# pytorch/torchsnapshot

Measured on AMD Instinct MI355X. Metric: checkpoint_save_GBps, higher is better.
Workload: dtype bf16; 1 GPU; model=llama-3-8b, model_bytes=16060522496, parallelism=fsdp1, storage=/tmp/tsamd_bench

## Files before the change

### torchsnapshot_amd/batcher.py

```python

from __future__ import annotations

import asyncio
from collections import defaultdict
from typing import Dict, List, Optional, Sequence

import torch

from . import knobs
from .io_types import (
    BufferConsumer,
    BufferStager,
    BufferType,
    ReadReq,
    StageContext,
    WriteReq,
)
from .io_preparers.tensor import TensorBufferStager
from .ops.staging import ALIGN, build_pack_items, get_pinned_pool, get_staging_engine
from .serialization import SERIALIZER_BUFFER


def _is_batchable(req: WriteReq) -> bool:
    stager = req.stager
    return (
        req.tensor_entry is not None
        and isinstance(stager, TensorBufferStager)
        and stager.serializer == SERIALIZER_BUFFER
        and not stager.tensor.is_quantized
        and stager.get_staging_cost_bytes() < knobs.get_slab_size_threshold_bytes()
    )


def batch_write_requests(
    write_reqs: List[WriteReq], rank: int = 0
) -> List[WriteReq]:
    if knobs.is_batching_disabled():
        return write_reqs
    out: List[WriteReq] = []
    groups: Dict[str, List[WriteReq]] = defaultdict(list)
    for req in write_reqs:
        if _is_batchable(req):
            groups[str(req.stager.tensor.device)].append(req)
        else:
            out.append(req)

    slab_limit = knobs.get_slab_size_threshold_bytes()
    seq = 0
    for device_str, members in groups.items():
        if len(members) == 1:
            out.extend(members)
            continue
        cur: List[WriteReq] = []
        cur_bytes = 0
        for req in members:
            nbytes = req.stager.stored_nbytes()
            aligned = (nbytes + ALIGN - 1) // ALIGN * ALIGN
            if cur and cur_bytes + aligned > slab_limit:
                out.append(_make_slab(device_str, cur, rank, seq))
                seq += 1
                cur, cur_bytes = [], 0
            cur.append(req)
            cur_bytes += aligned
        if len(cur) == 1:
            out.append(cur[0])
        elif cur:
            out.append(_make_slab(device_str, cur, rank, seq))
            seq += 1
    return out


def _make_slab(
    device_str: str, members: List[WriteReq], rank: int, seq: int
) -> WriteReq:
    slab_path = f"batched/{rank}-{seq}"
    tensors = [m.stager.tensor.detach() for m in members]
    out_dtypes = [m.stager.save_dtype for m in members]
    _, offsets, total = build_pack_items(tensors, out_dtypes)
    for m, off in zip(members, offsets):
        entry = m.tensor_entry
        nbytes = m.stager.stored_nbytes()
        entry.location = slab_path
        entry.byte_range = [off, off + nbytes]
    is_async = any(m.stager.is_async_snapshot for m in members)
    stager = BatchedBufferStager(
        tensors=tensors,
        total_bytes=total,
        is_async_snapshot=is_async,
        out_dtypes=out_dtypes,
    )
    return WriteReq(path=slab_path, stager=stager)


class BatchedBufferStager(BufferStager):
    def __init__(
        self,
        tensors: Sequence[torch.Tensor],
        total_bytes: int,
        is_async_snapshot: bool,
        out_dtypes: Optional[Sequence[Optional[torch.dtype]]] = None,
    ) -> None:
        self.tensors = tensors
        self.out_dtypes = (
            list(out_dtypes) if out_dtypes is not None else [None] * len(tensors)
        )
        self.total_bytes = total_bytes
        self.is_async_snapshot = is_async_snapshot
        self._staged_batch = None
        self._pinned_block = None
        self.precomputed_checksum = None
        self.member_checksums = None

    def get_staging_cost_bytes(self) -> int:
        return self.total_bytes

    async def stage_buffer(self, ctx: StageContext) -> BufferType:
        loop = asyncio.get_running_loop()
        device = self.tensors[0].device
        if device.type == "cuda":
            return await loop.run_in_executor(ctx.executor, self._stage_device)
        return await loop.run_in_executor(ctx.executor, self._stage_cpu)

    def _stage_device(self) -> BufferType:
        from . import integrity

        engine = get_staging_engine(self.tensors[0].device)
        ck = integrity.checksumming_enabled()
        batch = engine.stage(
            self.tensors, compute_checksums=ck, out_dtypes=self.out_dtypes
        )
        batch.wait()
        if ck and batch.checksums is not None:
            total = sum(batch.checksums) % (1 << 64)
            self.precomputed_checksum = "psum64:" + format(total, "016x")
            self.member_checksums = [
                (off, off + n, "psum64:" + format(v % (1 << 64), "016x"))
                for off, n, v in zip(
                    batch.offsets, batch.nbytes_list, batch.checksums
                )
            ]
        self._staged_batch = batch
        return batch.slab_memoryview()

    def _stage_cpu(self) -> BufferType:
        from . import integrity

        items, offsets, total = build_pack_items(self.tensors, self.out_dtypes)
        slab = bytearray(total)
        mv = memoryview(slab)
        from .serialization import tensor_as_memoryview

        ck = integrity.checksumming_enabled()
        members = []
        for t, off, out_dtype in zip(self.tensors, offsets, self.out_dtypes):
            if out_dtype is not None and out_dtype != t.dtype:
                t = t.to(out_dtype)
            nbytes = t.numel() * t.element_size()
            if nbytes == 0:
                continue
            src = tensor_as_memoryview(t if t.is_contiguous() else t.contiguous())
            mv[off : off + nbytes] = src
            if ck:
                members.append(
                    (
                        off,
                        off + nbytes,
                        integrity.psum64_hexdigest(src, word_base=off // 8),
                    )
                )
        if ck:
            self.member_checksums = members
            total_ck = sum(
                int(v[len("psum64:"):], 16) for _, _, v in members
            ) % (1 << 64)
            self.precomputed_checksum = "psum64:" + format(total_ck, "016x")
        return mv

    def release_buffer(self) -> None:
        if self._staged_batch is not None:
            self._staged_batch.release()
            self._staged_batch = None
        self.tensors = ()
        self.out_dtypes = []



_MERGE_GAP_BYTES = 4 * 1024 * 1024


def batch_read_requests(read_reqs: List[ReadReq]) -> List[ReadReq]:
    if knobs.is_batching_disabled():
        return read_reqs
    out: List[ReadReq] = []
    by_path: Dict[str, List[ReadReq]] = defaultdict(list)
    for rr in read_reqs:
        if rr.byte_range is not None:
            by_path[rr.path].append(rr)
        else:
            out.append(rr)

    limit = knobs.get_slab_size_threshold_bytes() * 2
    for path, members in by_path.items():
        if len(members) == 1:
            out.extend(members)
            continue
        members.sort(key=lambda r: r.byte_range[0])
        span: List[ReadReq] = []
        span_start = span_end = 0
        for rr in members:
            s, e = rr.byte_range
            if span and (s - span_end > _MERGE_GAP_BYTES or e - span_start > limit):
                out.append(_make_span(path, span, span_start, span_end))
                span = []
            if not span:
                span_start = s
            span.append(rr)
            span_end = max(span_end, e)
        if span:
            out.append(_make_span(path, span, span_start, span_end))
    return out


def _make_span(
    path: str, members: List[ReadReq], start: int, end: int
) -> ReadReq:
    if len(members) == 1:
        return members[0]
    consumer = BatchedBufferConsumer(members=members, span_start=start)
    return ReadReq(
        path=path,
        byte_range=(start, end),
        consumer=consumer,
        buf_alloc=(
            consumer.alloc_pinned_buffer
            if consumer._device_fast_path_target() is not None
            else None
        ),
    )


class BatchedBufferConsumer(BufferConsumer):
    def __init__(self, members: List[ReadReq], span_start: int) -> None:
        self.members = members
        self.span_start = span_start
        self._pinned_block = None
        self._pinned_nbytes = 0
        self.expected_psum = None

    def alloc_pinned_buffer(self, nbytes: int) -> memoryview:
        self._pinned_block = get_pinned_pool().acquire(max(nbytes, 1))
        self._pinned_nbytes = nbytes
        return memoryview(self._pinned_block.tensor.numpy())[:nbytes]

    def close(self) -> None:
        if self._pinned_block is not None:
            get_pinned_pool().release(self._pinned_block)
            self._pinned_block = None

    def get_consuming_cost_bytes(self) -> int:
        total = 0
        for m in self.members:
            total += m.consumer.get_consuming_cost_bytes()
        return total

    def _device_fast_path_target(self):
        device = None
        for m in self.members:
            getter = getattr(m.consumer, "device_span_target", None)
            target = getter() if getter else None
            if target is None:
                return None
            if device is None:
                device = target
            elif target != device:
                return None
        return device

    def will_verify_on_device(self) -> bool:
        from .ops.staging import HIP_EXT_AVAILABLE

        return HIP_EXT_AVAILABLE and self._device_fast_path_target() is not None

    async def consume_buffer(self, ctx: StageContext, buf: BufferType) -> None:
        device = self._device_fast_path_target()
        if device is None:
            mv = memoryview(buf)
            for m in self.members:
                s, e = m.byte_range
                sub = mv[s - self.span_start : e - self.span_start]
                await m.consumer.consume_buffer(ctx, sub)
            return

        def work() -> None:
            if self._pinned_block is not None:
                n = self._pinned_nbytes
                dev_span = self._pinned_block.tensor[:n].to(
                    device, non_blocking=False
                )
            else:
                mv = memoryview(buf)
                nbytes = mv.nbytes
                pool = get_pinned_pool()
                block = pool.acquire(max(nbytes, 1))
                try:
                    src = torch.frombuffer(mv, dtype=torch.uint8)
                    block.tensor[:nbytes].copy_(src)
                    dev_span = block.tensor[:nbytes].to(
                        device, non_blocking=False
                    )
                finally:
                    pool.release(block)
            if self.expected_psum is not None:
                from .ops.staging import verify_device_psum

                verify_device_psum(
                    dev_span,
                    self.expected_psum,
                    f"{self.members[0].path} span[{self.span_start}:"
                    f"{self.span_start + memoryview(buf).nbytes}]",
                )
            for m in self.members:
                s, e = m.byte_range
                sub = dev_span[s - self.span_start : e - self.span_start]
                m.consumer.consume_from_device_u8(sub)

        await asyncio.get_running_loop().run_in_executor(ctx.executor, work)
```

### torchsnapshot_amd/io_preparers/tensor.py

```python

from __future__ import annotations

import asyncio
from typing import Any, List, Optional, Tuple

import torch

from ..io_types import (
    BufferConsumer,
    BufferStager,
    BufferType,
    ReadReq,
    StageContext,
    WriteReq,
)
from ..manifest import TensorEntry
from ..serialization import (
    SERIALIZER_BUFFER,
    SERIALIZER_QTENSOR,
    SERIALIZER_TORCH_SAVE,
    dtype_to_str,
    pick_serializer,
    qtensor_as_bytes,
    qtensor_from_bytes,
    str_to_dtype,
    tensor_as_memoryview,
    tensor_from_memoryview,
    torch_load_from_bytes,
    torch_save_as_bytes,
)


class LoadFuture:

    __slots__ = ["obj"]

    def __init__(self, obj: Any = None) -> None:
        self.obj = obj


def tensor_copy(dst: torch.Tensor, src: torch.Tensor) -> None:
    dst = dst.detach()
    if src.is_quantized and not dst.is_quantized:
        src = src.dequantize()
    if dst.is_quantized and not src.is_quantized:
        raise ValueError(
            "cannot load a non-quantized payload into a quantized tensor "
            f"(dst dtype {dst.dtype})"
        )
    if (
        dst.is_quantized
        and src.is_quantized
        and dst.qscheme() != src.qscheme()
    ):
        raise ValueError(
            f"quantization scheme mismatch: dst {dst.qscheme()} vs src "
            f"{src.qscheme()}"
        )
    dst.copy_(src)


class TensorIOPreparer:
    @staticmethod
    def prepare_write(
        storage_path: str,
        tensor: torch.Tensor,
        replicated: bool = False,
        is_async_snapshot: bool = False,
        save_dtype: Optional[torch.dtype] = None,
    ) -> Tuple[TensorEntry, List[WriteReq]]:
        serializer = pick_serializer(tensor)
        if save_dtype == tensor.dtype:
            save_dtype = None
        if save_dtype is not None and serializer != SERIALIZER_BUFFER:
            raise ValueError(
                f"save_dtype={save_dtype} needs a buffer-serialized tensor, "
                f"got serializer '{serializer}' for dtype {tensor.dtype}"
            )
        entry = TensorEntry(
            location=storage_path,
            serializer=serializer,
            dtype=dtype_to_str(save_dtype or tensor.dtype),
            shape=list(tensor.shape),
            replicated=replicated,
        )
        stager = TensorBufferStager(
            tensor=tensor,
            serializer=serializer,
            is_async_snapshot=is_async_snapshot,
            save_dtype=save_dtype,
        )
        return entry, [
            WriteReq(path=storage_path, stager=stager, tensor_entry=entry)
        ]

    @staticmethod
    def prepare_read(
        entry: TensorEntry,
        tensor_out: Optional[torch.Tensor] = None,
        buffer_size_limit_bytes: Optional[int] = None,
    ) -> Tuple[List[ReadReq], LoadFuture]:
        nbytes = entry.nbytes_estimate()
        if (
            buffer_size_limit_bytes is not None
            and entry.serializer == SERIALIZER_BUFFER
            and entry.byte_range is None
            and nbytes > buffer_size_limit_bytes
        ):
            return TensorIOPreparer._prepare_read_tiled(
                entry, tensor_out, buffer_size_limit_bytes
            )
        fut = LoadFuture(tensor_out)
        consumer = TensorBufferConsumer(entry=entry, tensor_out=tensor_out, fut=fut)
        byte_range = tuple(entry.byte_range) if entry.byte_range else None
        buf_alloc = (
            consumer.alloc_pinned_buffer
            if (
                tensor_out is not None
                and tensor_out.device.type == "cuda"
                and entry.serializer == SERIALIZER_BUFFER
            )
            else None
        )
        return [
            ReadReq(
                path=entry.location,
                consumer=consumer,
                byte_range=byte_range,
                buf_alloc=buf_alloc,
            )
        ], fut

    @staticmethod
    def _prepare_read_tiled(
        entry: TensorEntry,
        tensor_out: Optional[torch.Tensor],
        limit: int,
    ) -> Tuple[List[ReadReq], LoadFuture]:
        dtype = str_to_dtype(entry.dtype)
        nbytes = entry.nbytes_estimate()
        elem = max(dtype.itemsize, 1)
        direct = (
            tensor_out is not None
            and tensor_out.is_contiguous()
            and tensor_out.dtype == dtype
        )
        staging = (
            tensor_out
            if direct
            else torch.empty(entry.shape, dtype=dtype)
        )
        fut = LoadFuture(tensor_out if tensor_out is not None else staging)
        flat_u8 = staging.reshape(-1).view(torch.uint8) if nbytes else None
        tile = max(limit - limit % elem, elem)
        reqs: List[ReadReq] = []
        state = _TiledReadState(
            remaining=(nbytes + tile - 1) // tile if nbytes else 0,
            staging=staging,
            tensor_out=None if direct else tensor_out,
        )
        for start in range(0, nbytes, tile):
            end = min(start + tile, nbytes)
            consumer = _TensorTileConsumer(
                dst_flat_u8=flat_u8, start=start, end=end, state=state
            )
            reqs.append(
                ReadReq(
                    path=entry.location,
                    byte_range=(start, end),
                    consumer=consumer,
                    buf_alloc=(
                        consumer.alloc_pinned_buffer
                        if staging.device.type == "cuda"
                        else None
                    ),
                )
            )
        if not reqs:
            if tensor_out is not None and not direct:
                tensor_copy(tensor_out, staging)
        return reqs, fut


class _TiledReadState:
    def __init__(
        self,
        remaining: int,
        staging: torch.Tensor,
        tensor_out: Optional[torch.Tensor],
    ) -> None:
        self.remaining = remaining
        self.staging = staging
        self.tensor_out = tensor_out
        self.lock = __import__("threading").Lock()


class _TensorTileConsumer(BufferConsumer):
    def __init__(
        self,
        dst_flat_u8: torch.Tensor,
        start: int,
        end: int,
        state: _TiledReadState,
    ) -> None:
        self.dst_flat_u8 = dst_flat_u8
        self.start = start
        self.end = end
        self.state = state
        self._pinned_block = None

    def alloc_pinned_buffer(self, nbytes: int) -> memoryview:
        from ..ops.staging import get_pinned_pool

        self._pinned_block = get_pinned_pool().acquire(max(nbytes, 1))
        return memoryview(self._pinned_block.tensor.numpy())[:nbytes]

    def close(self) -> None:
        if self._pinned_block is not None:
            from ..ops.staging import get_pinned_pool

            get_pinned_pool().release(self._pinned_block)
            self._pinned_block = None

    def get_consuming_cost_bytes(self) -> int:
        return self.end - self.start

    async def consume_buffer(self, ctx: StageContext, buf: BufferType) -> None:
        def work() -> None:
            n = self.end - self.start
            if self._pinned_block is not None:
                src = self._pinned_block.tensor[:n]
            else:
                src = torch.frombuffer(buf, dtype=torch.uint8)
            self.dst_flat_u8[self.start : self.end].copy_(src)
            with self.state.lock:
                self.state.remaining -= 1
                last = self.state.remaining == 0
            if last and self.state.tensor_out is not None:
                tensor_copy(self.state.tensor_out, self.state.staging)

        await asyncio.get_running_loop().run_in_executor(ctx.executor, work)


class TensorBufferStager(BufferStager):
    def __init__(
        self,
        tensor: torch.Tensor,
        serializer: str,
        is_async_snapshot: bool = False,
        save_dtype: Optional[torch.dtype] = None,
    ) -> None:
        self.tensor = tensor
        self.serializer = serializer
        self.is_async_snapshot = is_async_snapshot
        self.save_dtype = save_dtype
        self._staged_batch = None
        self.precomputed_checksum = None

    def stored_nbytes(self) -> int:
        esz = (
            self.save_dtype.itemsize
            if self.save_dtype is not None
            else self.tensor.element_size()
        )
        return self.tensor.numel() * esz

    def get_staging_cost_bytes(self) -> int:
        nbytes = self.stored_nbytes()
        if self.serializer in (SERIALIZER_TORCH_SAVE, SERIALIZER_QTENSOR):
            return 2 * nbytes
        return nbytes

    async def stage_buffer(self, ctx: StageContext) -> BufferType:
        loop = asyncio.get_running_loop()
        if self.tensor.device.type == "cuda":
            return await loop.run_in_executor(ctx.executor, self._stage_device)
        return await loop.run_in_executor(ctx.executor, self._stage_cpu, ctx)

    def _stage_device(self) -> BufferType:
        from ..ops.staging import get_staging_engine
        from ..uvm_tensor import is_uvm_tensor, uvm_to_cpu

        t = self.tensor.detach()
        if t.is_quantized or self.serializer != SERIALIZER_BUFFER:
            cpu = t.cpu()
            if self.serializer == SERIALIZER_QTENSOR:
                return qtensor_as_bytes(cpu)
            return torch_save_as_bytes(cpu)
        if is_uvm_tensor(t):
            cpu = uvm_to_cpu(t)
            if self.save_dtype is not None:
                return tensor_as_memoryview(
                    cpu.to(self.save_dtype).contiguous()
                )
            if self.is_async_snapshot:
                cpu = cpu.clone()
            return tensor_as_memoryview(cpu.contiguous())
        from .. import integrity

        engine = get_staging_engine(t.device)
        ck = integrity.checksumming_enabled()
        batch = engine.stage(
            [t],
            compute_checksums=ck,
            out_dtypes=None if self.save_dtype is None else [self.save_dtype],
        )
        batch.wait()
        if ck and batch.checksums is not None:
            self.precomputed_checksum = "psum64:" + format(
                batch.checksums[0], "016x"
            )
        self._staged_batch = batch
        return batch.memoryview_of(0)

    def _stage_cpu(self, ctx: StageContext) -> BufferType:
        t = self.tensor.detach()
        if self.serializer == SERIALIZER_QTENSOR:
            return qtensor_as_bytes(t)
        if self.serializer == SERIALIZER_TORCH_SAVE:
            return torch_save_as_bytes(t)
        if self.save_dtype is not None:
            return tensor_as_memoryview(t.to(self.save_dtype).contiguous())
        if self._should_copy_cpu_tensor(t, ctx):
            t = t.contiguous().clone() if not t.is_contiguous() else t.clone()
        elif not t.is_contiguous():
            t = t.contiguous()
        return tensor_as_memoryview(t)

    def _should_copy_cpu_tensor(self, t: torch.Tensor, ctx: StageContext) -> bool:
        if self.is_async_snapshot:
            return True
        if t.numel() * t.element_size() != t.untyped_storage().nbytes():
            return True
        return False

    def release_buffer(self) -> None:
        if self._staged_batch is not None:
            self._staged_batch.release()
            self._staged_batch = None
        self.tensor = None


class TensorBufferConsumer(BufferConsumer):
    def __init__(
        self,
        entry: TensorEntry,
        tensor_out: Optional[torch.Tensor],
        fut: LoadFuture,
    ) -> None:
        self.entry = entry
        self.tensor_out = tensor_out
        self.fut = fut
        self._pinned_block = None
        self._pinned_nbytes = 0
        self.expected_psum = None

    def alloc_pinned_buffer(self, nbytes: int) -> memoryview:
        from ..ops.staging import get_pinned_pool

        self._pinned_block = get_pinned_pool().acquire(max(nbytes, 1))
        self._pinned_nbytes = nbytes
        return memoryview(self._pinned_block.tensor.numpy())[:nbytes]

    def close(self) -> None:
        if self._pinned_block is not None:
            from ..ops.staging import get_pinned_pool

            get_pinned_pool().release(self._pinned_block)
            self._pinned_block = None

    def get_consuming_cost_bytes(self) -> int:
        nbytes = self.entry.nbytes_estimate()
        if self.entry.serializer == SERIALIZER_TORCH_SAVE:
            return 2 * nbytes
        return nbytes

    def device_span_target(self):
        if (
            self.tensor_out is not None
            and self.tensor_out.device.type == "cuda"
            and self.entry.serializer == SERIALIZER_BUFFER
        ):
            return self.tensor_out.device
        return None

    def will_verify_on_device(self) -> bool:
        from ..ops.staging import HIP_EXT_AVAILABLE

        return (
            HIP_EXT_AVAILABLE
            and self._pinned_block is not None
            and self.tensor_out is not None
            and self.tensor_out.device.type == "cuda"
            and self.entry.serializer == SERIALIZER_BUFFER
        )

    def consume_from_device_u8(self, dev_u8: torch.Tensor) -> None:
        dtype = str_to_dtype(self.entry.dtype)
        loaded = (
            dev_u8.view(dtype).reshape(tuple(self.entry.shape))
            if dtype != torch.uint8
            else dev_u8.reshape(tuple(self.entry.shape))
        )
        tensor_copy(self.tensor_out, loaded)
        self.fut.obj = self.tensor_out

    async def consume_buffer(self, ctx: StageContext, buf: BufferType) -> None:
        def work() -> None:
            dtype = (
                str_to_dtype(self.entry.dtype)
                if self.entry.serializer == SERIALIZER_BUFFER
                else None
            )
            if self.entry.serializer == SERIALIZER_QTENSOR:
                loaded = qtensor_from_bytes(buf)
            elif self.entry.serializer == SERIALIZER_TORCH_SAVE:
                loaded = torch_load_from_bytes(bytes(buf))
            elif (
                self._pinned_block is not None
                and self.tensor_out is not None
                and self.tensor_out.device.type == "cuda"
            ):
                n = self._pinned_nbytes
                dev_u8 = self._pinned_block.tensor[:n].to(
                    self.tensor_out.device, non_blocking=False
                )
                if self.expected_psum is not None:
                    from ..ops.staging import verify_device_psum

                    verify_device_psum(
                        dev_u8, self.expected_psum, self.entry.location
                    )
                loaded = (
                    dev_u8.view(dtype).reshape(tuple(self.entry.shape))
                    if dtype != torch.uint8
                    else dev_u8.reshape(tuple(self.entry.shape))
                )
            elif (
                self.tensor_out is not None
                and self.tensor_out.device.type == "cuda"
            ):
                from ..ops.staging import copy_buffer_via_pinned

                loaded = copy_buffer_via_pinned(
                    buf,
                    dtype=dtype,
                    shape=tuple(self.entry.shape),
                    device=self.tensor_out.device,
                )
            else:
                loaded = tensor_from_memoryview(
                    memoryview(buf), dtype=dtype, shape=tuple(self.entry.shape)
                )
            if self.tensor_out is not None:
                tensor_copy(self.tensor_out, loaded)
                self.fut.obj = self.tensor_out
            else:
                self.fut.obj = loaded

        await asyncio.get_running_loop().run_in_executor(ctx.executor, work)
```

### torchsnapshot_amd/io_types.py

```python

from __future__ import annotations

import abc
from concurrent.futures import ThreadPoolExecutor
from dataclasses import dataclass, field
from typing import Any, Optional, Tuple

BufferType = Any


@dataclass
class StageContext:

    executor: ThreadPoolExecutor
    is_async: bool = False


class BufferStager(abc.ABC):
    @abc.abstractmethod
    async def stage_buffer(self, ctx: StageContext) -> BufferType:
        """Produce the serialized bytes for this write request."""

    @abc.abstractmethod
    def get_staging_cost_bytes(self) -> int:
        """Peak host-memory cost of staging this buffer (for budgeting)."""

    def release_buffer(self) -> None:
        """Called once the storage write completed; return pooled buffers."""


class BufferConsumer(abc.ABC):
    @abc.abstractmethod
    async def consume_buffer(self, ctx: StageContext, buf: BufferType) -> None:
        """Apply the read bytes to the destination object."""

    @abc.abstractmethod
    def get_consuming_cost_bytes(self) -> int:
        """Peak host-memory cost of holding + consuming this buffer."""

    def close(self) -> None:
        """Called when the pipeline is done with this request (success or
        failure); return pooled buffers here."""


@dataclass
class WriteReq:
    path: str
    stager: BufferStager
    tensor_entry: Optional[Any] = None


@dataclass
class ReadReq:
    path: str
    consumer: BufferConsumer
    byte_range: Optional[Tuple[int, int]] = None
    buf_alloc: Optional[Any] = None


@dataclass
class WriteIO:
    path: str
    buf: BufferType


@dataclass
class ReadIO:
    path: str
    byte_range: Optional[Tuple[int, int]] = None
    buf: Optional[BufferType] = field(default=None)
    buf_alloc: Optional[Any] = None


class StoragePlugin(abc.ABC):

    @abc.abstractmethod
    async def write(self, write_io: WriteIO) -> None:
        ...

    @abc.abstractmethod
    async def read(self, read_io: ReadIO) -> None:
        """Fill ``read_io.buf`` with the (byte-ranged) content of the path."""

    @abc.abstractmethod
    async def delete(self, path: str) -> None:
        ...

    async def delete_dir(self, path: str) -> None:
        raise NotImplementedError

    @abc.abstractmethod
    async def close(self) -> None:
        ...

    async def close_for_loop(self) -> None:
        """Release resources tied to the CURRENT event loop (called when a
        pipeline's loop ends). Backends holding per-loop sessions override
        this; default no-op."""


    def sync_write(self, write_io: WriteIO) -> None:
        from .scheduler import run_coro_sync

        run_coro_sync(self.write(write_io))

    def sync_read(self, read_io: ReadIO) -> None:
        from .scheduler import run_coro_sync

        run_coro_sync(self.read(read_io))

    def sync_close(self) -> None:
        from .scheduler import run_coro_sync

        run_coro_sync(self.close())
```

### torchsnapshot_amd/knobs.py

```python

from __future__ import annotations

import contextlib
import os
from typing import Iterator

_MB = 1024 * 1024


def _env_bytes(name: str, default: int) -> int:
    val = os.environ.get(name)
    if val is None:
        return default
    return int(float(val))


def _env_int(name: str, default: int) -> int:
    val = os.environ.get(name)
    if val is None:
        return default
    return int(val)


def _env_flag(name: str) -> bool:
    return os.environ.get(name, "0") not in ("0", "", "false", "False")



def get_max_chunk_size_bytes() -> int:
    return _env_bytes("TSAMD_MAX_CHUNK_SIZE_BYTES", 512 * _MB)


def get_max_shard_size_bytes() -> int:
    return _env_bytes("TSAMD_MAX_SHARD_SIZE_BYTES", 512 * _MB)


def get_slab_size_threshold_bytes() -> int:
    return _env_bytes("TSAMD_SLAB_SIZE_THRESHOLD_BYTES", 512 * _MB)


def is_batching_disabled() -> bool:
    return _env_flag("TSAMD_DISABLE_BATCHING")


def is_partitioner_disabled() -> bool:
    return _env_flag("TSAMD_DISABLE_PARTITIONER")



def get_max_io_concurrency() -> int:
    return _env_int("TSAMD_MAX_PER_RANK_IO_CONCURRENCY", 32)


def get_num_staging_threads() -> int:
    return _env_int("TSAMD_NUM_STAGING_THREADS", 8)


def get_memory_budget_override_bytes() -> int | None:
    val = os.environ.get("TSAMD_PER_RANK_MEMORY_BUDGET_BYTES")
    return None if val is None else int(float(val))


def get_pinned_block_size_bytes() -> int:
    return _env_bytes(
        "TSAMD_PINNED_BLOCK_SIZE_BYTES", max(get_max_chunk_size_bytes(), 512 * _MB)
    )


def get_pinned_pool_bytes() -> int:
    override = os.environ.get("TSAMD_PINNED_POOL_BYTES")
    if override is not None:
        return int(float(override))
    import psutil

    local_ws = int(os.environ.get("LOCAL_WORLD_SIZE", "1") or "1")
    total = psutil.virtual_memory().total
    return min(24 * 1024 * _MB, int(total * 0.35)) // max(local_ws, 1)


def get_pinned_block_count() -> int:
    override = os.environ.get("TSAMD_PINNED_BLOCK_COUNT")
    if override is not None:
        return int(override)
    return max(get_pinned_pool_bytes() // get_pinned_block_size_bytes(), 2)


def is_hip_staging_disabled() -> bool:
    return _env_flag("TSAMD_DISABLE_HIP_STAGING")


def get_async_shadow_mode() -> str:
    val = os.environ.get("TSAMD_ASYNC_SHADOW", "auto").lower()
    return val if val in ("auto", "1", "0") else "auto"


def get_shadow_cpu_max_bytes() -> int:
    return _env_bytes("TSAMD_SHADOW_CPU_MAX_BYTES", 1024 * _MB)


def get_storage_write_chunk_bytes() -> int:
    return _env_bytes("TSAMD_FS_WRITE_CHUNK_BYTES", 256 * _MB)


def is_fs_reuse_pages_enabled() -> bool:
    return os.environ.get("TSAMD_FS_REUSE_PAGES", "1") not in (
        "0", "", "false", "False"
    )


def get_fs_parallel_io_min_bytes() -> int:
    return _env_bytes("TSAMD_FS_PARALLEL_IO_MIN_BYTES", 128 * _MB)


def get_fs_io_segment_bytes() -> int:
    return _env_bytes("TSAMD_FS_IO_SEGMENT_BYTES", 64 * _MB)



def is_sharded_elasticity_root_only() -> bool:
    return _env_flag("TSAMD_ENABLE_SHARDED_TENSOR_ELASTICITY_ROOT_ONLY")



@contextlib.contextmanager
def override_env(name: str, value: str) -> Iterator[None]:
    prev = os.environ.get(name)
    os.environ[name] = value
    try:
        yield
    finally:
        if prev is None:
            os.environ.pop(name, None)
        else:
            os.environ[name] = prev


def override_max_chunk_size_bytes(nbytes: int):
    return override_env("TSAMD_MAX_CHUNK_SIZE_BYTES", str(nbytes))


def override_max_shard_size_bytes(nbytes: int):
    return override_env("TSAMD_MAX_SHARD_SIZE_BYTES", str(nbytes))


def override_slab_size_threshold_bytes(nbytes: int):
    return override_env("TSAMD_SLAB_SIZE_THRESHOLD_BYTES", str(nbytes))


def override_batching_disabled(disabled: bool):
    return override_env("TSAMD_DISABLE_BATCHING", "1" if disabled else "0")


def override_max_io_concurrency(n: int):
    return override_env("TSAMD_MAX_PER_RANK_IO_CONCURRENCY", str(n))
```

### torchsnapshot_amd/ops/hip/file_sink.h

```cpp

#pragma once

#include <cerrno>
#include <cstddef>
#include <cstdint>
#include <string>

#include <fcntl.h>
#include <sys/stat.h>
#include <sys/types.h>
#include <unistd.h>

namespace tsamd {

constexpr size_t kReuseMinBytes = 1u << 20;

struct SinkResult {
  int err = 0;
  const char* op = "";
  bool reused = false;
};

namespace detail {

inline int close_noeintr(int fd) {
  int r = ::close(fd);
  return (r != 0 && errno != EINTR) ? errno : 0;
}

inline int fsync_dir_of(const std::string& path) {
  std::string dir;
  size_t slash = path.find_last_of('/');
  if (slash == std::string::npos) dir = ".";
  else if (slash == 0) dir = "/";
  else dir = path.substr(0, slash);
  int dfd = ::open(dir.c_str(), O_RDONLY | O_DIRECTORY | O_CLOEXEC);
  if (dfd < 0) return errno;
  int err = 0;
  if (::fsync(dfd) != 0) err = errno;
  int cerr = close_noeintr(dfd);
  return err ? err : cerr;
}

}

inline SinkResult file_write(const std::string& path, const void* data,
                             size_t nbytes, bool do_fsync, size_t chunk_bytes,
                             bool reuse) {
  SinkResult res;
  if (chunk_bytes == 0) {
    res.err = EINVAL;
    res.op = "chunk_bytes";
    return res;
  }
  int fd = -1;
  off_t old_size = 0;
  if (reuse && nbytes >= kReuseMinBytes) {
    fd = ::open(path.c_str(), O_WRONLY | O_CLOEXEC);
    if (fd >= 0) {
      struct stat st;
      if (::fstat(fd, &st) != 0) {
        res.err = errno;
        res.op = "fstat";
        (void)detail::close_noeintr(fd);
        return res;
      }
      if (S_ISREG(st.st_mode)) {
        old_size = st.st_size;
        res.reused = true;
      } else {
        (void)detail::close_noeintr(fd);
        fd = -1;
      }
    } else if (errno != ENOENT) {
      res.err = errno;
      res.op = "open";
      return res;
    }
  }
  if (fd < 0) {
    fd = ::open(path.c_str(), O_WRONLY | O_CREAT | O_TRUNC | O_CLOEXEC, 0644);
    if (fd < 0) {
      res.err = errno;
      res.op = "open";
      return res;
    }
  }

  const char* p = static_cast<const char*>(data);
  size_t off = 0;
  while (off < nbytes) {
    size_t want = nbytes - off < chunk_bytes ? nbytes - off : chunk_bytes;
    ssize_t n = ::pwrite(fd, p + off, want, static_cast<off_t>(off));
    if (n < 0) {
      if (errno == EINTR) continue;
      res.err = errno;
      res.op = "pwrite";
      break;
    }
    if (n == 0) {
      res.err = EIO;
      res.op = "pwrite";
      break;
    }
    off += static_cast<size_t>(n);
  }
  if (!res.err && res.reused && old_size > static_cast<off_t>(nbytes)) {
    int r;
    do {
      r = ::ftruncate(fd, static_cast<off_t>(nbytes));
    } while (r != 0 && errno == EINTR);
    if (r != 0) {
      res.err = errno;
      res.op = "ftruncate";
    }
  }
  if (!res.err && do_fsync) {
    if (::fsync(fd) != 0) {
      res.err = errno;
      res.op = "fsync";
    } else if (int derr = detail::fsync_dir_of(path)) {
      res.err = derr;
      res.op = "fsync(dir)";
    }
  }
  int cerr = detail::close_noeintr(fd);
  if (!res.err && cerr) {
    res.err = cerr;
    res.op = "close";
  }
  return res;
}

}
```

### torchsnapshot_amd/ops/hip/staging.hip

```cpp

#include <hip/hip_runtime.h>
#include <pybind11/pybind11.h>
#include <pybind11/stl.h>

#include <cstdint>
#include <cstring>
#include <mutex>
#include <stdexcept>
#include <string>
#include <thread>
#include <unordered_map>
#include <vector>

#include "file_sink.h"

namespace py = pybind11;

#define HIP_CHECK(expr)                                                     \
  do {                                                                      \
    hipError_t _e = (expr);                                                 \
    if (_e != hipSuccess) {                                                 \
      throw std::runtime_error(std::string("HIP error at " #expr ": ") +    \
                               hipGetErrorString(_e));                      \
    }                                                                       \
  } while (0)

namespace {

constexpr int kMaxDims = 6;
constexpr uint32_t kWorkUnitBytes = 64 * 1024;
constexpr int kBlockThreads = 256;
constexpr uint32_t kWideRowBytes = 2048;

struct Desc {
  const char* tensor_base;
  unsigned long long flat_off;
  uint32_t nbytes;
  uint32_t row_bytes;
  uint32_t vec;
  uint32_t ndim;
  uint32_t sizes[kMaxDims];
  long long strides[kMaxDims];
  uint32_t cast;
};

constexpr uint32_t kCastNone = 0;
constexpr uint32_t kCastBF16 = 1;
constexpr uint32_t kCastF16 = 2;


__device__ __host__ inline unsigned long long psum_mult(unsigned long long w) {
  unsigned long long z = w + 0x9E3779B97F4A7C15ull;
  z = (z ^ (z >> 30)) * 0xBF58476D1CE4E5B9ull;
  z = (z ^ (z >> 27)) * 0x94D049BB133111EBull;
  z = z ^ (z >> 31);
  return z | 1ull;
}

template <int VEC>
__device__ inline unsigned long long psum_contrib(
    const char* bytes, unsigned long long file_off) {
  unsigned long long acc = 0;
  if (VEC == 16) {
    const unsigned long long* p = reinterpret_cast<const unsigned long long*>(bytes);
    unsigned long long w = file_off >> 3;
    acc += p[0] * psum_mult(w);
    acc += p[1] * psum_mult(w + 1);
  } else if (VEC == 8) {
    acc += *reinterpret_cast<const unsigned long long*>(bytes) *
           psum_mult(file_off >> 3);
  } else {
    unsigned long long v = 0;
    if (VEC == 4) v = *reinterpret_cast<const uint32_t*>(bytes);
    else if (VEC == 2) v = *reinterpret_cast<const uint16_t*>(bytes);
    else v = *reinterpret_cast<const unsigned char*>(bytes);
    acc += (v << (8 * (file_off & 7))) * psum_mult(file_off >> 3);
  }
  return acc;
}

__device__ inline unsigned long long row_offset(const Desc& d, uint32_t row) {
  unsigned long long off = 0;
  uint32_t rem = row;
#pragma unroll
  for (int k = kMaxDims - 1; k >= 0; --k) {
    if (k >= (int)d.ndim) continue;
    uint32_t sz = d.sizes[k];
    uint32_t idx = rem % sz;
    rem /= sz;
    off += (unsigned long long)idx * (unsigned long long)d.strides[k];
  }
  return off;
}

template <int VEC, bool GATHER>
__device__ inline void copy_vec(char* flat, const char* strided) {
  if (GATHER) {
    if (VEC == 16)
      *reinterpret_cast<uint4*>(flat) = *reinterpret_cast<const uint4*>(strided);
    else if (VEC == 8)
      *reinterpret_cast<uint64_t*>(flat) = *reinterpret_cast<const uint64_t*>(strided);
    else if (VEC == 4)
      *reinterpret_cast<uint32_t*>(flat) = *reinterpret_cast<const uint32_t*>(strided);
    else if (VEC == 2)
      *reinterpret_cast<uint16_t*>(flat) = *reinterpret_cast<const uint16_t*>(strided);
    else
      *flat = *strided;
  } else {
    if (VEC == 16)
      *reinterpret_cast<uint4*>(const_cast<char*>(strided)) = *reinterpret_cast<const uint4*>(flat);
    else if (VEC == 8)
      *reinterpret_cast<uint64_t*>(const_cast<char*>(strided)) = *reinterpret_cast<const uint64_t*>(flat);
    else if (VEC == 4)
      *reinterpret_cast<uint32_t*>(const_cast<char*>(strided)) = *reinterpret_cast<const uint32_t*>(flat);
    else if (VEC == 2)
      *reinterpret_cast<uint16_t*>(const_cast<char*>(strided)) = *reinterpret_cast<const uint16_t*>(flat);
    else
      *const_cast<char*>(strided) = *flat;
  }
}

template <int VEC, bool GATHER, bool HASH>
__device__ unsigned long long process_range(const Desc& d, char* flat_base,
                                            uint32_t s, uint32_t e) {
  char* flat = flat_base + d.flat_off;
  const uint32_t tid = threadIdx.x;
  const uint32_t rb = d.row_bytes;
  unsigned long long h = 0;
  if (d.ndim == 0 || rb == d.nbytes) {
    const char* src = d.tensor_base;
    for (uint32_t i = s + tid * VEC; i < e; i += kBlockThreads * VEC) {
      copy_vec<VEC, GATHER>(flat + i, src + i);
      if (HASH) h += psum_contrib<VEC>(src + i, d.flat_off + i);
    }
    return h;
  }
  if (rb >= kWideRowBytes) {
    uint32_t row = s / rb;
    uint32_t col = s - row * rb;
    uint32_t off = s;
    while (off < e) {
      const char* src = d.tensor_base + row_offset(d, row);
      uint32_t n = min(rb - col, e - off);
      for (uint32_t i = tid * VEC; i < n; i += kBlockThreads * VEC) {
        copy_vec<VEC, GATHER>(flat + off + i, src + col + i);
        if (HASH) h += psum_contrib<VEC>(src + col + i, d.flat_off + off + i);
      }
      off += n;
      ++row;
      col = 0;
    }
  } else {
    uint32_t first_row = s / rb;
    uint32_t last_row = (e - 1) / rb;
    for (uint32_t r = first_row + tid; r <= last_row; r += kBlockThreads) {
      const char* src = d.tensor_base + row_offset(d, r);
      uint32_t flat_pos = r * rb;
      uint32_t lo = flat_pos < s ? (s - flat_pos) : 0;
      uint32_t hi = (flat_pos + rb > e) ? (e - flat_pos) : rb;
      for (uint32_t i = lo; i < hi; i += VEC) {
        copy_vec<VEC, GATHER>(flat + flat_pos + i, src + i);
        if (HASH) h += psum_contrib<VEC>(src + i, d.flat_off + flat_pos + i);
      }
    }
  }
  return h;
}


__device__ __host__ inline uint32_t f32_to_bf16_bits(uint32_t u) {
  if ((u & 0x7FFFFFFFu) > 0x7F800000u) {
    return (u >> 16) | 0x0040u;
  }
  return (u + 0x7FFFu + ((u >> 16) & 1u)) >> 16;
}

__device__ __host__ inline uint32_t f32_to_f16_bits(uint32_t u) {
  const uint32_t sign = (u >> 16) & 0x8000u;
  const uint32_t a = u & 0x7FFFFFFFu;
  if (a > 0x7F800000u) return sign | 0x7E00u;
  if (a >= 0x47800000u) return sign | 0x7C00u;
  if (a >= 0x38800000u) {
    uint32_t r = a - 0x38000000u;
    r += 0x0FFFu + ((r >> 13) & 1u);
    return sign | (r >> 13);
  }
  if (a < 0x33000000u) return sign;
  const uint32_t mant = (a & 0x007FFFFFu) | 0x00800000u;
  const uint32_t shift = 126u - (a >> 23);
  uint32_t h = mant >> shift;
  const uint32_t rem = mant & ((1u << shift) - 1u);
  const uint32_t half = 1u << (shift - 1u);
  if (rem > half || (rem == half && (h & 1u))) ++h;
  return sign | h;
}

__device__ inline uint32_t cast_pair(uint32_t lo, uint32_t hi, uint32_t code) {
  if (code == kCastBF16) {
    return (f32_to_bf16_bits(lo) & 0xFFFFu) | (f32_to_bf16_bits(hi) << 16);
  }
  return f32_to_f16_bits(lo) | (f32_to_f16_bits(hi) << 16);
}

template <int VEC, bool HASH>
__device__ inline unsigned long long cast_vec(char* flat, const char* src,
                                              uint32_t code,
                                              unsigned long long file_off) {
  unsigned long long h = 0;
  if (VEC == 16) {
    const uint4 a = *reinterpret_cast<const uint4*>(src);
    const uint4 b = *reinterpret_cast<const uint4*>(src + 16);
    uint4 o;
    o.x = cast_pair(a.x, a.y, code);
    o.y = cast_pair(a.z, a.w, code);
    o.z = cast_pair(b.x, b.y, code);
    o.w = cast_pair(b.z, b.w, code);
    *reinterpret_cast<uint4*>(flat) = o;
    if (HASH) {
      unsigned long long w = file_off >> 3;
      h += (((unsigned long long)o.y << 32) | o.x) * psum_mult(w);
      h += (((unsigned long long)o.w << 32) | o.z) * psum_mult(w + 1);
    }
  } else if (VEC == 8) {
    const uint4 a = *reinterpret_cast<const uint4*>(src);
    uint2 o;
    o.x = cast_pair(a.x, a.y, code);
    o.y = cast_pair(a.z, a.w, code);
    *reinterpret_cast<uint2*>(flat) = o;
    if (HASH) {
      h += (((unsigned long long)o.y << 32) | o.x) * psum_mult(file_off >> 3);
    }
  } else if (VEC == 4) {
    const uint2 a = *reinterpret_cast<const uint2*>(src);
    const uint32_t o = cast_pair(a.x, a.y, code);
    *reinterpret_cast<uint32_t*>(flat) = o;
    if (HASH) {
      h += ((unsigned long long)o << (8 * (file_off & 7))) *
           psum_mult(file_off >> 3);
    }
  } else {
    const uint32_t a = *reinterpret_cast<const uint32_t*>(src);
    const uint32_t o = (code == kCastBF16 ? f32_to_bf16_bits(a)
                                          : f32_to_f16_bits(a)) & 0xFFFFu;
    *reinterpret_cast<uint16_t*>(flat) = (uint16_t)o;
    if (HASH) {
      h += ((unsigned long long)o << (8 * (file_off & 7))) *
           psum_mult(file_off >> 3);
    }
  }
  return h;
}

template <int VEC, bool HASH>
__device__ unsigned long long process_range_cast(const Desc& d,
                                                 char* flat_base, uint32_t s,
                                                 uint32_t e) {
  char* flat = flat_base + d.flat_off;
  const uint32_t tid = threadIdx.x;
  const uint32_t rb = d.row_bytes;
  const uint32_t code = d.cast;
  unsigned long long h = 0;
  if (d.ndim == 0 || rb == d.nbytes) {
    const char* src = d.tensor_base;
    for (uint32_t i = s + tid * VEC; i < e; i += kBlockThreads * VEC) {
      h += cast_vec<VEC, HASH>(flat + i, src + 2ull * i, code, d.flat_off + i);
    }
    return h;
  }
  if (rb >= kWideRowBytes) {
    uint32_t row = s / rb;
    uint32_t col = s - row * rb;
    uint32_t off = s;
    while (off < e) {
      const char* src = d.tensor_base + row_offset(d, row) + 2ull * col;
      uint32_t n = min(rb - col, e - off);
      for (uint32_t i = tid * VEC; i < n; i += kBlockThreads * VEC) {
        h += cast_vec<VEC, HASH>(flat + off + i, src + 2ull * i, code,
                                 d.flat_off + off + i);
      }
      off += n;
      ++row;
      col = 0;
    }
  } else {
    uint32_t first_row = s / rb;
    uint32_t last_row = (e - 1) / rb;
    for (uint32_t r = first_row + tid; r <= last_row; r += kBlockThreads) {
      const char* src = d.tensor_base + row_offset(d, r);
      uint32_t flat_pos = r * rb;
      uint32_t lo = flat_pos < s ? (s - flat_pos) : 0;
      uint32_t hi = (flat_pos + rb > e) ? (e - flat_pos) : rb;
      for (uint32_t i = lo; i < hi; i += VEC) {
        h += cast_vec<VEC, HASH>(flat + flat_pos + i, src + 2ull * i, code,
                                 d.flat_off + flat_pos + i);
      }
    }
  }
  return h;
}

template <bool GATHER, bool HASH, bool CAST = false>
__global__ __launch_bounds__(kBlockThreads) void pack_kernel(
    const Desc* __restrict__ descs, int n,
    const unsigned long long* __restrict__ wu_prefix,
    unsigned long long total_wus, char* __restrict__ flat_base,
    unsigned long long* __restrict__ hash_out) {
  for (unsigned long long wu = blockIdx.x; wu < total_wus; wu += gridDim.x) {
    int lo = 0, hi = n - 1;
    while (lo < hi) {
      int mid = (lo + hi + 1) >> 1;
      if (wu_prefix[mid] <= wu) lo = mid;
      else hi = mid - 1;
    }
    const Desc d = descs[lo];
    unsigned long long local_wu = wu - wu_prefix[lo];
    uint32_t s = (uint32_t)(local_wu * kWorkUnitBytes);
    uint32_t e = s + kWorkUnitBytes > d.nbytes ? d.nbytes
                                               : s + kWorkUnitBytes;
    unsigned long long h = 0;
    if (CAST && d.cast != kCastNone) {
      switch (d.vec) {
        case 16: h = process_range_cast<16, HASH>(d, flat_base, s, e); break;
        case 8: h = process_range_cast<8, HASH>(d, flat_base, s, e); break;
        case 4: h = process_range_cast<4, HASH>(d, flat_base, s, e); break;
        default: h = process_range_cast<2, HASH>(d, flat_base, s, e); break;
      }
    } else {
      switch (d.vec) {
        case 16: h = process_range<16, GATHER, HASH>(d, flat_base, s, e); break;
        case 8: h = process_range<8, GATHER, HASH>(d, flat_base, s, e); break;
        case 4: h = process_range<4, GATHER, HASH>(d, flat_base, s, e); break;
        case 2: h = process_range<2, GATHER, HASH>(d, flat_base, s, e); break;
        default: h = process_range<1, GATHER, HASH>(d, flat_base, s, e); break;
      }
    }
    if (HASH) {
      for (int delta = 32; delta > 0; delta >>= 1) {
        h += __shfl_down(h, delta, 64);
      }
      if ((threadIdx.x & 63) == 0 && h != 0) {
        atomicAdd(&hash_out[lo], h);
      }
    }
  }
}


struct DeviceCtx {
  hipStream_t d2h_stream = nullptr;
  hipStream_t h2d_stream = nullptr;
  hipStream_t verify_stream = nullptr;
};

struct Op {
  hipEvent_t ev = nullptr;
  int device = 0;
  void* scratch = nullptr;
  std::vector<char> host_staging;
};

std::mutex g_mu;
std::unordered_map<int, DeviceCtx> g_ctx;
std::unordered_map<long long, Op> g_ops;
long long g_next_handle = 1;

DeviceCtx& get_ctx(int device) {
  std::lock_guard<std::mutex> lk(g_mu);
  auto it = g_ctx.find(device);
  if (it == g_ctx.end()) {
    HIP_CHECK(hipSetDevice(device));
    DeviceCtx ctx;
    HIP_CHECK(hipStreamCreateWithFlags(&ctx.d2h_stream, hipStreamNonBlocking));
    HIP_CHECK(hipStreamCreateWithFlags(&ctx.h2d_stream, hipStreamNonBlocking));
    it = g_ctx.emplace(device, ctx).first;
  }
  return it->second;
}

long long register_op(hipEvent_t ev, int device, void* scratch,
                      std::vector<char>&& staging) {
  std::lock_guard<std::mutex> lk(g_mu);
  long long h = g_next_handle++;
  Op op;
  op.ev = ev;
  op.device = device;
  op.scratch = scratch;
  op.host_staging = std::move(staging);
  g_ops.emplace(h, std::move(op));
  return h;
}

void chain_after(hipStream_t side, uintptr_t producer_stream, int device) {
  hipEvent_t dep;
  HIP_CHECK(hipEventCreateWithFlags(&dep, hipEventDisableTiming));
  hipError_t e =
      hipEventRecord(dep, reinterpret_cast<hipStream_t>(producer_stream));
  if (e == hipSuccess) {
    e = hipStreamWaitEvent(side, dep, 0);
  }
  (void)hipEventDestroy(dep);
  if (e != hipSuccess) {
    throw std::runtime_error(std::string("HIP error chaining streams: ") +
                             hipGetErrorString(e));
  }
}

constexpr int kRowInts = 19;

std::vector<Desc> parse_descs(const std::vector<unsigned long long>& flat,
                              int n) {
  if ((int)flat.size() != n * kRowInts) {
    throw std::runtime_error("bad descriptor array length");
  }
  std::vector<Desc> descs(n);
  for (int i = 0; i < n; ++i) {
    const unsigned long long* r = flat.data() + i * kRowInts;
    Desc& d = descs[i];
    d.tensor_base = reinterpret_cast<const char*>(r[0]);
    d.flat_off = r[1];
    if (r[2] >= (1ull << 32)) {
      throw std::runtime_error(
          "tensor too large for pack kernel (>=4GB); chunk it upstream");
    }
    d.nbytes = (uint32_t)r[2];
    d.row_bytes = (uint32_t)r[3];
    d.vec = (uint32_t)r[4];
    d.ndim = (uint32_t)r[5];
    for (int k = 0; k < kMaxDims; ++k) {
      d.sizes[k] = (uint32_t)r[6 + k];
      d.strides[k] = (long long)r[12 + k];
    }
    if (d.ndim > (uint32_t)kMaxDims) {
      throw std::runtime_error("too many outer dims");
    }
    if (r[18] > kCastF16) {
      throw std::runtime_error("unknown cast code in descriptor");
    }
    d.cast = (uint32_t)r[18];
    if (d.cast != kCastNone && d.nbytes != 0) {
      const uint32_t v = d.vec;
      if (v != 16 && v != 8 && v != 4 && v != 2) {
        throw std::runtime_error("cast descriptor: vec must be 16/8/4/2");
      }
      if (d.row_bytes == 0 || d.row_bytes % v != 0 ||
          d.nbytes % d.row_bytes != 0) {
        throw std::runtime_error("cast descriptor: row_bytes/vec mismatch");
      }
      const unsigned long long src_align = v == 16 ? 16 : 2ull * v;
      bool ok = (r[0] % src_align) == 0;
      for (uint32_t k = 0; k < d.ndim; ++k) {
        ok = ok && ((unsigned long long)d.strides[k] % src_align) == 0;
      }
      if (!ok) {
        throw std::runtime_error(
            "cast descriptor: source not aligned for its vec");
      }
    }
  }
  return descs;
}

long long launch_pack(const std::vector<unsigned long long>& flat, int n,
                      uintptr_t slab_ptr, uintptr_t pinned_ptr,
                      unsigned long long total_bytes, uintptr_t producer_stream,
                      int device, bool gather, uintptr_t hash_out_ptr) {
  HIP_CHECK(hipSetDevice(device));
  DeviceCtx& ctx = get_ctx(device);
  hipStream_t stream = gather ? ctx.d2h_stream : ctx.h2d_stream;

  std::vector<Desc> descs = parse_descs(flat, n);
  bool any_cast = false;
  for (const Desc& d : descs) any_cast = any_cast || d.cast != kCastNone;
  if (any_cast && !gather) {
    throw std::runtime_error(
        "scatter_h2d does not support cast descriptors (gather only)");
  }
  std::vector<unsigned long long> wu_prefix(n + 1, 0);
  for (int i = 0; i < n; ++i) {
    unsigned long long wus =
        (descs[i].nbytes + kWorkUnitBytes - 1) / kWorkUnitBytes;
    wu_prefix[i + 1] = wu_prefix[i] + wus;
  }
  unsigned long long total_wus = wu_prefix[n];

  char* flat_base;
  if (slab_ptr != 0) {
    flat_base = reinterpret_cast<char*>(slab_ptr);
  } else {
    void* dev_ptr = nullptr;
    hipError_t err = hipHostGetDevicePointer(
        &dev_ptr, reinterpret_cast<void*>(pinned_ptr), 0);
    flat_base = reinterpret_cast<char*>(
        err == hipSuccess && dev_ptr ? dev_ptr
                                     : reinterpret_cast<void*>(pinned_ptr));
  }

  chain_after(stream, producer_stream, device);

  size_t desc_bytes = sizeof(Desc) * n;
  size_t prefix_bytes = sizeof(unsigned long long) * (n + 1);
  std::vector<char> staging(desc_bytes + prefix_bytes);
  memcpy(staging.data(), descs.data(), desc_bytes);
  memcpy(staging.data() + desc_bytes, wu_prefix.data(), prefix_bytes);
  void* scratch = nullptr;
  HIP_CHECK(hipMallocAsync(&scratch, staging.size(), stream));
  HIP_CHECK(hipMemcpyAsync(scratch, staging.data(), staging.size(),
                           hipMemcpyHostToDevice, stream));

  const Desc* d_descs = reinterpret_cast<const Desc*>(scratch);
  const unsigned long long* d_prefix =
      reinterpret_cast<const unsigned long long*>(
          reinterpret_cast<char*>(scratch) + desc_bytes);

  if (!gather && slab_ptr != 0) {
    HIP_CHECK(hipMemcpyAsync(reinterpret_cast<void*>(slab_ptr),
                             reinterpret_cast<void*>(pinned_ptr), total_bytes,
                             hipMemcpyHostToDevice, stream));
  }

  bool direct_mode = (slab_ptr == 0);
  unsigned long long grid_cap = direct_mode ? 256ull : 16384ull;
  if (const char* env = getenv("TSAMD_PACK_GRID")) {
    long v = atol(env);
    if (v > 0) grid_cap = (unsigned long long)v;
  }
  unsigned int grid = (unsigned int)std::min<unsigned long long>(
      total_wus == 0 ? 1 : total_wus, grid_cap);
  unsigned long long* hash_out =
      reinterpret_cast<unsigned long long*>(hash_out_ptr);
  if (any_cast && hash_out != nullptr) {
    hipLaunchKernelGGL((pack_kernel<true, true, true>), dim3(grid),
                       dim3(kBlockThreads), 0, stream, d_descs, n, d_prefix,
                       total_wus, flat_base, hash_out);
  } else if (any_cast) {
    hipLaunchKernelGGL((pack_kernel<true, false, true>), dim3(grid),
                       dim3(kBlockThreads), 0, stream, d_descs, n, d_prefix,
                       total_wus, flat_base, nullptr);
  } else if (gather && hash_out != nullptr) {
    hipLaunchKernelGGL((pack_kernel<true, true>), dim3(grid),
                       dim3(kBlockThreads), 0, stream, d_descs, n, d_prefix,
                       total_wus, flat_base, hash_out);
  } else if (gather) {
    hipLaunchKernelGGL((pack_kernel<true, false>), dim3(grid),
                       dim3(kBlockThreads), 0, stream, d_descs, n, d_prefix,
                       total_wus, flat_base, nullptr);
  } else {
    hipLaunchKernelGGL((pack_kernel<false, false>), dim3(grid),
                       dim3(kBlockThreads), 0, stream, d_descs, n, d_prefix,
                       total_wus, flat_base, nullptr);
  }
  HIP_CHECK(hipGetLastError());

  if (gather && slab_ptr != 0) {
    HIP_CHECK(hipMemcpyAsync(reinterpret_cast<void*>(pinned_ptr),
                             reinterpret_cast<void*>(slab_ptr), total_bytes,
                             hipMemcpyDeviceToHost, stream));
  }
  HIP_CHECK(hipFreeAsync(scratch, stream));

  hipEvent_t ev;
  HIP_CHECK(hipEventCreateWithFlags(&ev, hipEventDisableTiming));
  HIP_CHECK(hipEventRecord(ev, stream));
  return register_op(ev, device, nullptr, std::move(staging));
}

}


static long long d2h_copy(uintptr_t src, uintptr_t dst_pinned,
                          unsigned long long nbytes, uintptr_t producer_stream,
                          int device) {
  HIP_CHECK(hipSetDevice(device));
  DeviceCtx& ctx = get_ctx(device);
  chain_after(ctx.d2h_stream, producer_stream, device);
  HIP_CHECK(hipMemcpyAsync(reinterpret_cast<void*>(dst_pinned),
                           reinterpret_cast<void*>(src), nbytes,
                           hipMemcpyDeviceToHost, ctx.d2h_stream));
  hipEvent_t ev;
  HIP_CHECK(hipEventCreateWithFlags(&ev, hipEventDisableTiming));
  HIP_CHECK(hipEventRecord(ev, ctx.d2h_stream));
  return register_op(ev, device, nullptr, {});
}

static long long h2d_copy(uintptr_t src_pinned, uintptr_t dst,
                          unsigned long long nbytes, uintptr_t producer_stream,
                          int device) {
  HIP_CHECK(hipSetDevice(device));
  DeviceCtx& ctx = get_ctx(device);
  chain_after(ctx.h2d_stream, producer_stream, device);
  HIP_CHECK(hipMemcpyAsync(reinterpret_cast<void*>(dst),
                           reinterpret_cast<void*>(src_pinned), nbytes,
                           hipMemcpyHostToDevice, ctx.h2d_stream));
  hipEvent_t ev;
  HIP_CHECK(hipEventCreateWithFlags(&ev, hipEventDisableTiming));
  HIP_CHECK(hipEventRecord(ev, ctx.h2d_stream));
  return register_op(ev, device, nullptr, {});
}

static long long pack_d2h(const std::vector<unsigned long long>& flat, int n,
                          uintptr_t slab_ptr, uintptr_t pinned_ptr,
                          unsigned long long total_bytes,
                          uintptr_t producer_stream, int device,
                          uintptr_t hash_out_ptr = 0) {
  return launch_pack(flat, n, slab_ptr, pinned_ptr, total_bytes,
                     producer_stream, device, true, hash_out_ptr);
}

static long long scatter_h2d(const std::vector<unsigned long long>& flat, int n,
                             uintptr_t slab_ptr, uintptr_t pinned_ptr,
                             unsigned long long total_bytes,
                             uintptr_t producer_stream, int device) {
  return launch_pack(flat, n, slab_ptr, pinned_ptr, total_bytes,
                     producer_stream, device, false, 0);
}


__global__ __launch_bounds__(kBlockThreads) void psum_flat_kernel(
    const char* base, unsigned long long nbytes, unsigned long long byte0,
    unsigned long long* out) {
  unsigned long long acc = 0;
  unsigned long long tid =
      (unsigned long long)blockIdx.x * blockDim.x + threadIdx.x;
  unsigned long long nthreads = (unsigned long long)gridDim.x * blockDim.x;
  unsigned long long nwords = nbytes >> 3;
  unsigned long long w0 = byte0 >> 3;
  const unsigned long long* words =
      reinterpret_cast<const unsigned long long*>(base);
  for (unsigned long long w = tid; w < nwords; w += nthreads) {
    acc += words[w] * psum_mult(w0 + w);
  }
  if (tid == 0) {
    for (unsigned long long b = nwords << 3; b < nbytes; ++b) {
      unsigned long long v = (unsigned char)base[b];
      acc += (v << (8 * ((byte0 + b) & 7))) * psum_mult((byte0 + b) >> 3);
    }
  }
  __shared__ unsigned long long sh[kBlockThreads];
  sh[threadIdx.x] = acc;
  __syncthreads();
  for (int s = kBlockThreads / 2; s > 0; s >>= 1) {
    if ((int)threadIdx.x < s) sh[threadIdx.x] += sh[threadIdx.x + s];
    __syncthreads();
  }
  if (threadIdx.x == 0) {
    atomicAdd(out, sh[0]);
  }
}

static unsigned long long psum64_dev(uintptr_t ptr, unsigned long long nbytes,
                                     unsigned long long byte0,
                                     uintptr_t producer_stream, int device) {
  if (byte0 % 8 != 0) {
    throw std::runtime_error("psum64_dev: byte0 must be 8-aligned");
  }
  if (ptr % 8 != 0) {
    throw std::runtime_error("psum64_dev: buffer must be 8-aligned");
  }
  HIP_CHECK(hipSetDevice(device));
  (void)producer_stream;
  hipStream_t stream;
  {
    DeviceCtx& ctx = get_ctx(device);
    std::lock_guard<std::mutex> lk(g_mu);
    if (ctx.verify_stream == nullptr) {
      HIP_CHECK(hipStreamCreateWithFlags(&ctx.verify_stream,
                                         hipStreamNonBlocking));
    }
    stream = ctx.verify_stream;
  }
  unsigned long long* out = nullptr;
  HIP_CHECK(hipMallocAsync(reinterpret_cast<void**>(&out), 8, stream));
  HIP_CHECK(hipMemsetAsync(out, 0, 8, stream));
  unsigned int grid = 2048;
  if (nbytes < (1u << 22)) grid = 64;
  hipLaunchKernelGGL(psum_flat_kernel, dim3(grid), dim3(kBlockThreads), 0,
                     stream, reinterpret_cast<const char*>(ptr), nbytes,
                     byte0, out);
  HIP_CHECK(hipGetLastError());
  unsigned long long host_out = 0;
  HIP_CHECK(hipMemcpyAsync(&host_out, out, 8, hipMemcpyDeviceToHost, stream));
  HIP_CHECK(hipFreeAsync(out, stream));
  HIP_CHECK(hipStreamSynchronize(stream));
  return host_out;
}

static unsigned long long psum64_host(py::buffer b,
                                      unsigned long long word_base) {
  py::buffer_info info = b.request();
  const unsigned char* base = static_cast<const unsigned char*>(info.ptr);
  unsigned long long nbytes =
      (unsigned long long)info.size * (unsigned long long)info.itemsize;
  unsigned long long nwords = nbytes >> 3;
  unsigned int nthreads = std::thread::hardware_concurrency();
  if (nthreads == 0) nthreads = 4;
  if (nwords < (1u << 16)) nthreads = 1;
  std::vector<unsigned long long> partial(nthreads, 0);
  std::vector<std::thread> workers;
  unsigned long long per = nwords / nthreads;
  py::gil_scoped_release release;
  for (unsigned int t = 0; t < nthreads; ++t) {
    unsigned long long lo = t * per;
    unsigned long long hi = (t + 1 == nthreads) ? nwords : lo + per;
    workers.emplace_back([=, &partial]() {
      unsigned long long acc = 0;
      const unsigned long long* w =
          reinterpret_cast<const unsigned long long*>(base);
      for (unsigned long long i = lo; i < hi; ++i) {
        unsigned long long v;
        memcpy(&v, w + i, 8);
        acc += v * psum_mult(word_base + i);
      }
      partial[t] = acc;
    });
  }
  for (auto& th : workers) th.join();
  unsigned long long total = 0;
  for (auto p : partial) total += p;
  for (unsigned long long bpos = nwords << 3; bpos < nbytes; ++bpos) {
    unsigned long long v = base[bpos];
    unsigned long long file_b = (word_base << 3) + bpos;
    total += (v << (8 * (file_b & 7))) * psum_mult(file_b >> 3);
  }
  return total;
}

static bool file_write(py::object path, py::object buf, bool fsync,
                       long long chunk_bytes, bool reuse) {
  if (chunk_bytes <= 0) {
    throw py::value_error("file_write: chunk_bytes must be positive");
  }
  PyObject* fs_bytes = nullptr;
  if (!PyUnicode_FSConverter(path.ptr(), &fs_bytes)) {
    throw py::error_already_set();
  }
  std::string cpath(PyBytes_AS_STRING(fs_bytes),
                    (size_t)PyBytes_GET_SIZE(fs_bytes));
  Py_DECREF(fs_bytes);
  Py_buffer view;
  if (PyObject_GetBuffer(buf.ptr(), &view, PyBUF_SIMPLE) != 0) {
    throw py::error_already_set();
  }
  tsamd::SinkResult res;
  {
    py::gil_scoped_release release;
    res = tsamd::file_write(cpath, view.buf, (size_t)view.len, fsync,
                            (size_t)chunk_bytes, reuse);
  }
  PyBuffer_Release(&view);
  if (res.err) {
    errno = res.err;
    PyErr_SetFromErrnoWithFilenameObject(PyExc_OSError, path.ptr());
    throw py::error_already_set();
  }
  return res.reused;
}

static void op_wait(long long handle) {
  hipEvent_t ev = nullptr;
  int device = 0;
  {
    std::lock_guard<std::mutex> lk(g_mu);
    auto it = g_ops.find(handle);
    if (it == g_ops.end()) return;
    ev = it->second.ev;
    device = it->second.device;
  }
  hipError_t e;
  {
    py::gil_scoped_release release;
    e = hipEventSynchronize(ev);
  }
  {
    std::lock_guard<std::mutex> lk(g_mu);
    auto it = g_ops.find(handle);
    if (it != g_ops.end()) {
      (void)hipEventDestroy(it->second.ev);
      g_ops.erase(it);
    }
  }
  if (e != hipSuccess) {
    throw std::runtime_error(std::string("hipEventSynchronize: ") +
                             hipGetErrorString(e));
  }
}

static bool op_query(long long handle) {
  std::lock_guard<std::mutex> lk(g_mu);
  auto it = g_ops.find(handle);
  if (it == g_ops.end()) return true;
  return hipEventQuery(it->second.ev) == hipSuccess;
}

static bool is_managed_ptr(uintptr_t ptr) {
  hipPointerAttribute_t attr;
  hipError_t e =
      hipPointerGetAttributes(&attr, reinterpret_cast<void*>(ptr));
  if (e != hipSuccess) {
    (void)hipGetLastError();
    return false;
  }
  return attr.type == hipMemoryTypeManaged;
}

static int device_count() {
  int n = 0;
  if (hipGetDeviceCount(&n) != hipSuccess) return 0;
  return n;
}


static uintptr_t managed_alloc(unsigned long long nbytes, int device) {
  HIP_CHECK(hipSetDevice(device));
  void* ptr = nullptr;
  HIP_CHECK(hipMallocManaged(&ptr, nbytes, hipMemAttachGlobal));
  return reinterpret_cast<uintptr_t>(ptr);
}

static void managed_free(uintptr_t ptr) {
  HIP_CHECK(hipFree(reinterpret_cast<void*>(ptr)));
}

static void managed_advise_preferred_cpu(uintptr_t ptr,
                                         unsigned long long nbytes) {
  hipError_t e = hipMemAdvise(reinterpret_cast<void*>(ptr), nbytes,
                              hipMemAdviseSetPreferredLocation,
                              hipCpuDeviceId);
  (void)e;
}

static void managed_prefetch(uintptr_t ptr, unsigned long long nbytes,
                             int device) {
  DeviceCtx& ctx = get_ctx(device >= 0 ? device : 0);
  hipError_t e = hipMemPrefetchAsync(
      reinterpret_cast<void*>(ptr), nbytes,
      device >= 0 ? device : hipCpuDeviceId, ctx.h2d_stream);
  (void)e;
  (void)hipStreamSynchronize(ctx.h2d_stream);
}

PYBIND11_MODULE(_csnap, m) {
  m.doc() = "torchsnapshot_amd HIP staging engine (gfx950)";
  m.def("d2h_copy", &d2h_copy, "async D2H copy on the side stream");
  m.def("h2d_copy", &h2d_copy, "async H2D copy on the side stream");
  m.def("pack_d2h", &pack_d2h,
        "gather-pack tensors into a slab and copy it to pinned host memory",
        py::arg("flat"), py::arg("n"), py::arg("slab_ptr"),
        py::arg("pinned_ptr"), py::arg("total_bytes"),
        py::arg("producer_stream"), py::arg("device"),
        py::arg("hash_out_ptr") = 0);
  m.def("scatter_h2d", &scatter_h2d,
        "copy pinned host bytes to device and scatter into strided tensors");
  m.def("psum64_host", &psum64_host,
        "single-pass threaded host psum64 of a buffer",
        py::arg("buf"), py::arg("word_base") = 0);
  m.def("psum64_dev", &psum64_dev,
        "psum64 of a flat contiguous device buffer (blocking)",
        py::arg("ptr"), py::arg("nbytes"), py::arg("byte0"),
        py::arg("producer_stream"), py::arg("device"));
  m.def("file_write", &file_write,
        "write a buffer to a file (GIL released); reuse=True overwrites an "
        "existing file of >= 1 MiB payload in place instead of truncating",
        py::arg("path"), py::arg("buf"), py::arg("fsync") = false,
        py::arg("chunk_bytes") = 256ll * 1024 * 1024, py::arg("reuse") = true);
  m.def("wait", &op_wait, "block until an op completes");
  m.def("query", &op_query, "poll an op");
  m.def("is_managed_ptr", &is_managed_ptr);
  m.def("device_count", &device_count);
  m.def("managed_alloc", &managed_alloc, "hipMallocManaged");
  m.def("managed_free", &managed_free);
  m.def("managed_advise_preferred_cpu", &managed_advise_preferred_cpu);
  m.def("managed_prefetch", &managed_prefetch);
}
```

### torchsnapshot_amd/ops/staging.py

```python

from __future__ import annotations

import math
import threading
from dataclasses import dataclass
from typing import Dict, List, Optional, Sequence, Tuple

import torch

from .. import knobs

ALIGN = 256

try:
    from torchsnapshot_amd import _csnap

    HIP_EXT_AVAILABLE = True
except ImportError:
    _csnap = None
    HIP_EXT_AVAILABLE = False


def _require_ext() -> None:
    if not HIP_EXT_AVAILABLE:
        raise RuntimeError(
            "torchsnapshot_amd's HIP staging extension (_csnap) is not built "
            "but a device tensor needs staging. Build it with "
            "`python -m torchsnapshot_amd.ops.build` (gfx950), or set "
            "TSAMD_DISABLE_HIP_STAGING=1 to explicitly use the slow torch "
            "fallback."
        )




def collapse_layout(t: torch.Tensor) -> Tuple[List[int], List[int]]:
    sizes = [s for s, st in zip(t.shape, t.stride()) if s != 1]
    strides = [st for s, st in zip(t.shape, t.stride()) if s != 1]
    if not sizes:
        return [1], [1]
    merged_sizes: List[int] = [sizes[0]]
    merged_strides: List[int] = [strides[0]]
    for s, st in zip(sizes[1:], strides[1:]):
        if merged_strides[-1] == st * s:
            merged_sizes[-1] *= s
            merged_strides[-1] = st
        else:
            merged_sizes.append(s)
            merged_strides.append(st)
    return merged_sizes, merged_strides


@dataclass
class PackItem:

    src_ptr: int
    flat_offset: int
    nbytes: int
    row_bytes: int
    outer_sizes: List[int]
    outer_strides: List[int]
    vec: int
    cast: int = 0


CAST_NONE = 0
CAST_F32_TO_BF16 = 1
CAST_F32_TO_F16 = 2

_CAST_CODES = {
    (torch.float32, torch.bfloat16): CAST_F32_TO_BF16,
    (torch.float32, torch.float16): CAST_F32_TO_F16,
}


def cast_code(src: torch.dtype, dst: Optional[torch.dtype]) -> int:
    if dst is None or dst == src:
        return CAST_NONE
    code = _CAST_CODES.get((src, dst))
    if code is None:
        raise ValueError(
            f"the gather kernel cannot cast {src} to {dst}; supported: "
            "float32 -> bfloat16, float32 -> float16"
        )
    return code


def build_pack_items(
    tensors: Sequence[torch.Tensor],
    out_dtypes: Optional[Sequence[Optional[torch.dtype]]] = None,
) -> Tuple[List[PackItem], List[int], int]:
    if out_dtypes is None:
        out_dtypes = [None] * len(tensors)
    if len(out_dtypes) != len(tensors):
        raise ValueError("out_dtypes must have one entry per tensor")
    items: List[PackItem] = []
    offsets: List[int] = []
    off = 0
    for t, out_dtype in zip(tensors, out_dtypes):
        cast = cast_code(t.dtype, out_dtype)
        if cast != CAST_NONE:
            item = _build_cast_item(t, out_dtype, cast, off)
            items.append(item)
            offsets.append(off)
            off += (item.nbytes + ALIGN - 1) // ALIGN * ALIGN
            continue
        nbytes = t.numel() * t.element_size()
        sizes, strides = collapse_layout(t)
        esz = t.element_size()
        if t.numel() == 0:
            items.append(PackItem(t.data_ptr(), off, 0, 0, [], [], 1))
            offsets.append(off)
            continue
        if strides and strides[-1] == 1:
            row_elems = sizes[-1]
            outer_sizes = sizes[:-1]
            outer_strides_b = [st * esz for st in strides[:-1]]
        else:
            row_elems = 1
            outer_sizes = sizes
            outer_strides_b = [st * esz for st in strides]
        row_bytes = row_elems * esz
        vec = 16
        vec = math.gcd(vec, row_bytes)
        vec = math.gcd(vec, t.data_ptr())
        for st in outer_strides_b:
            vec = math.gcd(vec, st if st else 16)
        items.append(
            PackItem(
                src_ptr=t.data_ptr(),
                flat_offset=off,
                nbytes=nbytes,
                row_bytes=row_bytes,
                outer_sizes=outer_sizes,
                outer_strides=outer_strides_b,
                vec=vec,
            )
        )
        offsets.append(off)
        off += (nbytes + ALIGN - 1) // ALIGN * ALIGN
    return items, offsets, off


def _build_cast_item(
    t: torch.Tensor, out_dtype: torch.dtype, cast: int, off: int
) -> PackItem:
    if t.numel() == 0:
        return PackItem(t.data_ptr(), off, 0, 0, [], [], 1, CAST_NONE)
    src_esz = t.element_size()
    dst_esz = out_dtype.itemsize
    sizes, strides = collapse_layout(t)
    if strides[-1] == 1:
        row_elems = sizes[-1]
        outer_sizes = sizes[:-1]
        outer_strides_b = [st * src_esz for st in strides[:-1]]
    else:
        row_elems = 1
        outer_sizes = sizes
        outer_strides_b = [st * src_esz for st in strides]
    row_bytes = row_elems * dst_esz
    src_align = math.gcd(16, t.data_ptr())
    for st in outer_strides_b:
        src_align = math.gcd(src_align, st if st else 16)
    if src_align < src_esz:
        raise ValueError(
            f"cannot cast-stage a {t.dtype} tensor whose address or strides "
            f"are not {src_esz}-byte aligned"
        )
    vec = min(math.gcd(16, row_bytes), 16 if src_align == 16 else src_align // 2)
    return PackItem(
        src_ptr=t.data_ptr(),
        flat_offset=off,
        nbytes=t.numel() * dst_esz,
        row_bytes=row_bytes,
        outer_sizes=outer_sizes,
        outer_strides=outer_strides_b,
        vec=vec,
        cast=cast,
    )


def _items_to_flat(items: List[PackItem]) -> List[int]:
    MAXD = 6
    flat: List[int] = []
    for it in items:
        if len(it.outer_sizes) > MAXD:
            raise ValueError(
                f"tensor layout too complex to pack ({len(it.outer_sizes)} "
                "outer dims after collapsing; max 6)"
            )
        row = [
            it.src_ptr,
            it.flat_offset,
            it.nbytes,
            it.row_bytes,
            it.vec,
            len(it.outer_sizes),
        ]
        sizes = list(it.outer_sizes) + [1] * (MAXD - len(it.outer_sizes))
        strides = list(it.outer_strides) + [0] * (MAXD - len(it.outer_strides))
        row += sizes + strides
        row.append(it.cast)
        flat += row
    return flat




class PinnedBlock:
    def __init__(self, tensor: torch.Tensor, pooled: bool) -> None:
        self.tensor = tensor
        self.pooled = pooled

    @property
    def nbytes(self) -> int:
        return self.tensor.numel()


class PinnedPool:

    def __init__(
        self, block_size: Optional[int] = None, block_count: Optional[int] = None
    ) -> None:
        self.block_size = block_size or knobs.get_pinned_block_size_bytes()
        self.max_blocks = block_count or knobs.get_pinned_block_count()
        self._free: List[torch.Tensor] = []
        self._allocated = 0
        self._cond = threading.Condition()

    def acquire(self, nbytes: int) -> PinnedBlock:
        if nbytes > self.block_size:
            return PinnedBlock(
                torch.empty(nbytes, dtype=torch.uint8, pin_memory=True),
                pooled=False,
            )
        with self._cond:
            while True:
                if self._free:
                    return PinnedBlock(self._free.pop(), pooled=True)
                if self._allocated < self.max_blocks:
                    self._allocated += 1
                    break
                self._cond.wait()
        return PinnedBlock(
            torch.empty(self.block_size, dtype=torch.uint8, pin_memory=True),
            pooled=True,
        )

    def release(self, block: PinnedBlock) -> None:
        if not block.pooled:
            return
        with self._cond:
            self._free.append(block.tensor)
            self._cond.notify()

    def prealloc_one(self) -> bool:
        with self._cond:
            if self._allocated >= self.max_blocks:
                return False
            self._allocated += 1
        tensor = torch.empty(self.block_size, dtype=torch.uint8, pin_memory=True)
        with self._cond:
            self._free.append(tensor)
            self._cond.notify()
        return True


_pool_lock = threading.Lock()
_pool: Optional[PinnedPool] = None


def get_pinned_pool() -> PinnedPool:
    global _pool
    with _pool_lock:
        if _pool is None:
            _pool = PinnedPool()
        return _pool


_warm_stop = threading.Event()
_warm_thread: Optional[threading.Thread] = None


def _join_warm_thread() -> None:
    _warm_stop.set()
    t = _warm_thread
    if t is not None and t.is_alive():
        t.join(timeout=30)


def warm_pinned_pool(nbytes: Optional[int] = None, background: bool = True) -> None:
    global _warm_thread
    pool = get_pinned_pool()

    def work() -> None:
        import os

        if nbytes is not None:
            target = nbytes
        else:
            target = min(
                pool.block_size * pool.max_blocks,
                int(float(os.environ.get("TSAMD_POOL_WARM_BYTES", 8 * 1024**3))),
            )
        allocated = 0
        while (
            not _warm_stop.is_set()
            and allocated < target
            and pool.prealloc_one()
        ):
            allocated += pool.block_size

    if background:
        import atexit

        with _pool_lock:
            if _warm_thread is not None and _warm_thread.is_alive():
                return
            _warm_thread = threading.Thread(
                target=work, name="tsamd-pool-warm", daemon=True
            )
            atexit.register(_join_warm_thread)
            _warm_thread.start()
    else:
        work()




@dataclass
class StagedBatch:

    pinned: PinnedBlock
    offsets: List[int]
    nbytes_list: List[int]
    total_bytes: int
    _handle: Optional[int] = None
    _device_slab: Optional[torch.Tensor] = None
    checksums: Optional[List[int]] = None
    _hash_tensor: Optional[torch.Tensor] = None
    _sources: Optional[Sequence[torch.Tensor]] = None
    _done: bool = False

    def wait(self) -> None:
        if self._done:
            return
        if self._handle is not None:
            _csnap.wait(self._handle)
            self._handle = None
        if self._hash_tensor is not None:
            self.checksums = [int(v) for v in self._hash_tensor.cpu().tolist()]
            self._hash_tensor = None
        self._device_slab = None
        self._sources = None
        self._done = True

    def memoryview_of(self, index: int) -> memoryview:
        assert self._done, "wait() before reading staged buffers"
        off = self.offsets[index]
        n = self.nbytes_list[index]
        if n == 0:
            return memoryview(b"")
        return memoryview(self.pinned.tensor.numpy())[off : off + n]

    def slab_memoryview(self) -> memoryview:
        assert self._done
        return memoryview(self.pinned.tensor.numpy())[: self.total_bytes]

    def release(self) -> None:
        get_pinned_pool().release(self.pinned)


class StagingEngine:

    def __init__(self, device: torch.device) -> None:
        self.device = device
        self._use_ext = HIP_EXT_AVAILABLE and not knobs.is_hip_staging_disabled()
        if not self._use_ext and not knobs.is_hip_staging_disabled():
            _require_ext()
        warm_pinned_pool()

    def stage(
        self,
        tensors: Sequence[torch.Tensor],
        compute_checksums: bool = False,
        out_dtypes: Optional[Sequence[Optional[torch.dtype]]] = None,
    ) -> StagedBatch:
        tensors = [
            t
            if (
                t.is_contiguous()
                or (
                    t.numel() * t.element_size() < 2**31
                    and all(s >= 0 for s in t.stride())
                )
            )
            else t.contiguous()
            for t in tensors
        ]
        items, offsets, total = build_pack_items(tensors, out_dtypes)
        nbytes_list = [it.nbytes for it in items]
        pinned = get_pinned_pool().acquire(max(total, 1))
        batch = StagedBatch(
            pinned=pinned,
            offsets=offsets,
            nbytes_list=nbytes_list,
            total_bytes=total,
        )
        if total == 0:
            batch._done = True
            return batch
        batch._sources = tensors
        try:
            if self._use_ext:
                self._stage_ext(
                    tensors, items, batch, total,
                    compute_checksums=compute_checksums,
                )
            else:
                self._stage_torch_fallback(tensors, items, batch, out_dtypes)
        except BaseException:
            get_pinned_pool().release(pinned)
            raise
        return batch


    def _stage_ext(
        self,
        tensors: Sequence[torch.Tensor],
        items: List[PackItem],
        batch: StagedBatch,
        total: int,
        compute_checksums: bool = False,
    ) -> None:
        dev_index = self.device.index or 0
        with torch.cuda.device(dev_index):
            cur_stream = torch.cuda.current_stream().cuda_stream
            single_contig = (
                len(items) == 1
                and not items[0].outer_sizes
                and items[0].cast == CAST_NONE
                and not compute_checksums
            )
            if single_contig:
                handle = _csnap.d2h_copy(
                    items[0].src_ptr,
                    batch.pinned.tensor.data_ptr(),
                    items[0].nbytes,
                    cur_stream,
                    dev_index,
                )
            else:
                mode = _pack_mode()
                slab = None
                slab_ptr = 0
                hash_ptr = 0
                if compute_checksums:
                    batch._hash_tensor = torch.zeros(
                        len(items), dtype=torch.uint64, device=self.device
                    )
                    hash_ptr = batch._hash_tensor.data_ptr()
                if mode == "slab":
                    slab = (
                        torch.zeros(total, dtype=torch.uint8, device=self.device)
                        if compute_checksums
                        else torch.empty(
                            total, dtype=torch.uint8, device=self.device
                        )
                    )
                    slab_ptr = slab.data_ptr()
                elif compute_checksums:
                    pin_np = batch.pinned.tensor.numpy()
                    prev_end = 0
                    for it in items:
                        if it.flat_offset > prev_end:
                            pin_np[prev_end : it.flat_offset] = 0
                        prev_end = it.flat_offset + it.nbytes
                    if total > prev_end:
                        pin_np[prev_end:total] = 0
                handle = _csnap.pack_d2h(
                    _items_to_flat(items),
                    len(items),
                    slab_ptr,
                    batch.pinned.tensor.data_ptr(),
                    total,
                    cur_stream,
                    dev_index,
                    hash_ptr,
                )
                batch._device_slab = slab
            batch._handle = handle


    def _stage_torch_fallback(
        self,
        tensors: Sequence[torch.Tensor],
        items: List[PackItem],
        batch: StagedBatch,
        out_dtypes: Optional[Sequence[Optional[torch.dtype]]] = None,
    ) -> None:
        if out_dtypes is None:
            out_dtypes = [None] * len(items)
        for t, it, out_dtype in zip(tensors, items, out_dtypes):
            if it.nbytes == 0:
                continue
            if it.cast != CAST_NONE:
                t = t.to(out_dtype)
            flat = t.contiguous().reshape(-1).view(torch.uint8)
            dst = batch.pinned.tensor[it.flat_offset : it.flat_offset + it.nbytes]
            dst.copy_(flat, non_blocking=True)
        torch.cuda.synchronize(self.device)
        batch._done = True


def _pack_mode() -> str:
    import os

    mode = os.environ.get("TSAMD_STAGE_MODE", "direct")
    if mode not in ("slab", "direct"):
        raise ValueError(f"TSAMD_STAGE_MODE must be slab|direct, got {mode}")
    return mode


def copy_buffer_via_pinned(
    buf, dtype: torch.dtype, shape: Sequence[int], device: torch.device
) -> torch.Tensor:
    mv = memoryview(buf)
    nbytes = mv.nbytes
    pool = get_pinned_pool()
    block = pool.acquire(max(nbytes, 1))
    try:
        src = torch.frombuffer(mv, dtype=torch.uint8)
        block.tensor[:nbytes].copy_(src)
        dev_u8 = block.tensor[:nbytes].to(device, non_blocking=False)
    finally:
        pool.release(block)
    if dtype == torch.uint8:
        return dev_u8.reshape(tuple(shape))
    return dev_u8.view(dtype).reshape(tuple(shape))


def device_psum64(dev_u8: torch.Tensor, file_byte_off: int = 0) -> int:
    _require_ext()
    assert dev_u8.dtype == torch.uint8 and dev_u8.is_contiguous()
    assert dev_u8.device.type == "cuda"
    if dev_u8.numel() == 0:
        return 0
    return int(
        _csnap.psum64_dev(
            dev_u8.data_ptr(),
            dev_u8.numel(),
            file_byte_off,
            torch.cuda.current_stream(dev_u8.device).cuda_stream,
            dev_u8.device.index,
        )
    )


def verify_device_psum(
    dev_u8: torch.Tensor, expected: "tuple[int, int]", what: str
) -> None:
    value, word_base = expected
    got = device_psum64(dev_u8, word_base * 8)
    if got != value:
        raise RuntimeError(
            f"checksum mismatch for '{what}': snapshot recorded "
            f"psum64:{value:016x}, device read back psum64:{got:016x} — "
            "the file is corrupted or was modified after the snapshot "
            "was committed"
        )


_engines: Dict[int, StagingEngine] = {}
_engines_lock = threading.Lock()


def get_staging_engine(device: torch.device) -> StagingEngine:
    idx = device.index if device.index is not None else torch.cuda.current_device()
    with _engines_lock:
        if idx not in _engines:
            _engines[idx] = StagingEngine(torch.device("cuda", idx))
        return _engines[idx]
```

### torchsnapshot_amd/scheduler.py

```python

from __future__ import annotations

import asyncio
import logging
import socket
import threading
import time
from concurrent.futures import ThreadPoolExecutor
from dataclasses import dataclass, field
from typing import Awaitable, Callable, List, Optional, TypeVar

import psutil

from . import knobs
from .io_types import ReadIO, ReadReq, StageContext, StoragePlugin, WriteIO, WriteReq
from .pg_wrapper import PGWrapper
from .roctx import roctx_range
from . import integrity

logger = logging.getLogger(__name__)

T = TypeVar("T")

_MAX_PER_RANK_MEMORY_BUDGET_BYTES = 32 * 1024 * 1024 * 1024
_AVAILABLE_MEMORY_FRACTION = 0.6


def run_coro_sync(coro: Awaitable[T]) -> T:
    try:
        asyncio.get_running_loop()
    except RuntimeError:
        return asyncio.run(coro)
    with ThreadPoolExecutor(max_workers=1) as ex:
        return ex.submit(asyncio.run, coro).result()


def get_local_world_size(pg: PGWrapper) -> int:
    hostnames: List[Optional[str]] = [None] * pg.get_world_size()
    pg.all_gather_object(hostnames, socket.gethostname())
    return hostnames.count(socket.gethostname())


def get_process_memory_budget_bytes(pg: PGWrapper) -> int:
    override = knobs.get_memory_budget_override_bytes()
    if override is not None:
        logger.info("Manual memory budget: %d bytes", override)
        return override
    available = psutil.virtual_memory().available
    budget = int(
        available * _AVAILABLE_MEMORY_FRACTION / max(get_local_world_size(pg), 1)
    )
    return min(budget, _MAX_PER_RANK_MEMORY_BUDGET_BYTES)


@dataclass
class ExecutionStats:
    total_reqs: int = 0
    staged_reqs: int = 0
    done_reqs: int = 0
    staged_bytes: int = 0
    io_bytes: int = 0
    stage_s: float = 0.0
    io_s: float = 0.0
    consume_s: float = 0.0
    begin_ts: float = field(default_factory=time.monotonic)
    staged_ts: Optional[float] = None
    end_ts: Optional[float] = None

    def throughput_bytes_per_sec(self) -> float:
        end = self.end_ts or time.monotonic()
        dur = max(end - self.begin_ts, 1e-9)
        return self.io_bytes / dur


class _Budget:

    def __init__(self, limit: int) -> None:
        self.limit = limit
        self.in_use = 0
        self.cond = asyncio.Condition()

    async def acquire(self, cost: int) -> None:
        async with self.cond:
            while not (
                self.in_use + cost <= self.limit
                or (self.in_use == 0 and cost > self.limit)
            ):
                await self.cond.wait()
            self.in_use += cost

    async def release(self, cost: int) -> None:
        async with self.cond:
            self.in_use -= cost
            self.cond.notify_all()


class PendingIOWork:

    def __init__(
        self,
        thread: threading.Thread,
        staged_event: threading.Event,
        done_event: threading.Event,
        stats: ExecutionStats,
        exc_holder: List[BaseException],
        checksums: Optional[dict] = None,
    ) -> None:
        self._thread = thread
        self._staged_event = staged_event
        self._done_event = done_event
        self.stats = stats
        self._exc_holder = exc_holder
        self.checksums = checksums if checksums is not None else {}
        self.sources_immutable = False

    def _maybe_raise(self) -> None:
        if self._exc_holder:
            raise self._exc_holder[0]

    def wait_staged(self) -> None:
        self._staged_event.wait()
        if not self._done_event.is_set():
            if self._exc_holder:
                self._thread.join()
                self._maybe_raise()
        else:
            self._maybe_raise()

    def complete(self) -> None:
        self._thread.join()
        self._maybe_raise()
        import os

        if os.environ.get("TSAMD_TIMING") and self.stats.staged_bytes:
            s = self.stats
            wall = (s.end_ts or 0) - s.begin_ts
            print(
                f"[tsamd timing] pipeline: wall={wall:.2f}s reqs={s.total_reqs} "
                f"staged={s.staged_bytes/1e9:.2f}GB stage_busy={s.stage_s:.2f}s "
                f"io_busy={s.io_s:.2f}s consume_busy={s.consume_s:.2f}s"
            )

    def done(self) -> bool:
        return self._done_event.is_set()


def _spawn_pipeline(
    main: Callable[[], Awaitable[None]],
    stats: ExecutionStats,
    staged_event: threading.Event,
    done_event: threading.Event,
    checksums: Optional[dict] = None,
) -> PendingIOWork:
    exc_holder: List[BaseException] = []

    def runner() -> None:
        try:
            asyncio.run(main())
        except BaseException as e:
            exc_holder.append(e)
        finally:
            stats.end_ts = time.monotonic()
            staged_event.set()
            done_event.set()

    thread = threading.Thread(
        target=runner, name="tsamd-io-pipeline", daemon=True
    )
    thread.start()
    return PendingIOWork(
        thread, staged_event, done_event, stats, exc_holder, checksums
    )




def execute_write_reqs(
    write_reqs: List[WriteReq],
    storage: StoragePlugin,
    memory_budget_bytes: int,
    rank: int,
    is_async: bool = False,
) -> PendingIOWork:
    stats = ExecutionStats(total_reqs=len(write_reqs))
    staged_event = threading.Event()
    done_event = threading.Event()
    checksums: dict = {}
    do_checksum = integrity.checksumming_enabled()

    ordered = sorted(
        write_reqs, key=lambda r: r.stager.get_staging_cost_bytes(), reverse=True
    )

    async def main() -> None:
        budget = _Budget(memory_budget_bytes)
        io_sem = asyncio.Semaphore(knobs.get_max_io_concurrency())
        staging_sem = asyncio.Semaphore(knobs.get_num_staging_threads() * 2)
        executor = ThreadPoolExecutor(
            max_workers=knobs.get_num_staging_threads(),
            thread_name_prefix="tsamd-stage",
        )
        ctx = StageContext(executor=executor, is_async=is_async)
        staged_remaining = len(ordered)
        all_staged = asyncio.Event()
        if staged_remaining == 0:
            all_staged.set()

        async def handle(req: WriteReq) -> None:
            nonlocal staged_remaining
            cost = req.stager.get_staging_cost_bytes()
            await budget.acquire(cost)
            try:
                async with staging_sem:
                    t0 = time.monotonic()
                    with roctx_range(f"tsamd:stage:{req.path}"):
                        buf = await req.stager.stage_buffer(ctx)
                    stats.stage_s += time.monotonic() - t0
                nbytes = memoryview(buf).nbytes
                if do_checksum:
                    pre = getattr(req.stager, "precomputed_checksum", None)
                    if pre is not None:
                        checksums[req.path] = pre
                    else:
                        checksums[req.path] = await asyncio.get_running_loop(
                        ).run_in_executor(
                            executor, integrity.psum64_hexdigest, buf
                        )
                    for s, e, v in (
                        getattr(req.stager, "member_checksums", None) or []
                    ):
                        checksums[integrity.member_key(req.path, s, e)] = v
                    checksums[integrity.len_key(req.path)] = str(nbytes)
                stats.staged_reqs += 1
                stats.staged_bytes += nbytes
                staged_remaining -= 1
                if staged_remaining == 0:
                    all_staged.set()
                async with io_sem:
                    t0 = time.monotonic()
                    with roctx_range(f"tsamd:write:{req.path}"):
                        await storage.write(WriteIO(path=req.path, buf=buf))
                    stats.io_s += time.monotonic() - t0
                stats.io_bytes += nbytes
                stats.done_reqs += 1
            finally:
                try:
                    req.stager.release_buffer()
                except Exception:
                    logger.exception("release_buffer failed for %s", req.path)
                await budget.release(cost)

        tasks = [asyncio.create_task(handle(r)) for r in ordered]
        reporter = asyncio.create_task(_report_progress(stats, rank, "write"))

        async def signal_staged() -> None:
            await all_staged.wait()
            stats.staged_ts = time.monotonic()
            staged_event.set()

        signaler = asyncio.create_task(signal_staged())
        try:
            results = await asyncio.gather(*tasks, return_exceptions=True)
            errors = [r for r in results if isinstance(r, BaseException)]
            if errors:
                raise errors[0]
        finally:
            signaler.cancel()
            reporter.cancel()
            executor.shutdown(wait=False)
            try:
                await storage.close_for_loop()
            except Exception:
                logger.exception("storage close at pipeline end failed")

    return _spawn_pipeline(main, stats, staged_event, done_event, checksums)


def sync_execute_write_reqs(
    write_reqs: List[WriteReq],
    storage: StoragePlugin,
    memory_budget_bytes: int,
    rank: int,
) -> ExecutionStats:
    pending = execute_write_reqs(
        write_reqs, storage, memory_budget_bytes, rank=rank, is_async=False
    )
    pending.complete()
    import os

    if os.environ.get("TSAMD_TIMING"):
        s = pending.stats
        wall = (s.end_ts or 0) - s.begin_ts
        print(
            f"[tsamd timing] write: wall={wall:.2f}s reqs={s.total_reqs} "
            f"bytes={s.io_bytes/1e9:.2f}GB stage_busy={s.stage_s:.2f}s "
            f"io_busy={s.io_s:.2f}s"
        )
    if rank == 0 and pending.stats.io_bytes:
        logger.info(
            "Wrote %.1f MB in %.2fs (%.2f GB/s)",
            pending.stats.io_bytes / 1e6,
            (pending.stats.end_ts or 0) - pending.stats.begin_ts,
            pending.stats.throughput_bytes_per_sec() / 1e9,
        )
    return pending.stats




def execute_read_reqs(
    read_reqs: List[ReadReq],
    storage: StoragePlugin,
    memory_budget_bytes: int,
    rank: int,
    checksums: Optional[dict] = None,
) -> PendingIOWork:
    stats = ExecutionStats(total_reqs=len(read_reqs))
    staged_event = threading.Event()
    done_event = threading.Event()

    ordered = sorted(
        read_reqs,
        key=lambda r: r.consumer.get_consuming_cost_bytes(),
        reverse=True,
    )

    async def main() -> None:
        budget = _Budget(memory_budget_bytes)
        io_sem = asyncio.Semaphore(knobs.get_max_io_concurrency())
        executor = ThreadPoolExecutor(
            max_workers=knobs.get_num_staging_threads(),
            thread_name_prefix="tsamd-consume",
        )
        ctx = StageContext(executor=executor)
        partial_sums: Dict[str, list] = {}

        async def handle(req: ReadReq) -> None:
            cost = req.consumer.get_consuming_cost_bytes()
            await budget.acquire(cost)
            try:
                read_io = ReadIO(
                    path=req.path,
                    byte_range=req.byte_range,
                    buf_alloc=req.buf_alloc,
                )
                async with io_sem:
                    t0 = time.monotonic()
                    await storage.read(read_io)
                    stats.io_s += time.monotonic() - t0
                buf = read_io.buf
                stats.io_bytes += memoryview(buf).nbytes
                if checksums:
                    loop = asyncio.get_running_loop()
                    dev_exp = None
                    try:
                        if req.consumer.will_verify_on_device():
                            if req.byte_range is None:
                                want = checksums.get(req.path, "")
                                if want.startswith("psum64:"):
                                    dev_exp = (int(want[7:], 16), 0)
                            else:
                                s0, e0 = req.byte_range
                                total = integrity.expected_span_psum(
                                    req.path, req.byte_range, checksums
                                )
                                if total is not None and s0 % 8 == 0:
                                    dev_exp = (total, s0 // 8)
                    except AttributeError:
                        pass
                    if dev_exp is not None:
                        req.consumer.expected_psum = dev_exp
                    elif req.byte_range is None:
                        await loop.run_in_executor(
                            executor, integrity.verify_buffer, req.path, buf,
                            checksums,
                        )
                    else:
                        verified = await loop.run_in_executor(
                            executor, integrity.verify_ranged_buffer,
                            req.path, buf, req.byte_range, checksums,
                        )
                        s, e = req.byte_range
                        whole = checksums.get(req.path, "")
                        if (
                            not verified
                            and whole.startswith("psum64:")
                            and s % 8 == 0
                        ):
                            val = await loop.run_in_executor(
                                executor, integrity.psum64_value, buf, s // 8
                            )
                            rec = partial_sums.setdefault(
                                req.path, [0, []]
                            )
                            rec[0] = (rec[0] + val) % (1 << 64)
                            rec[1].append((s, e))
                t0 = time.monotonic()
                await req.consumer.consume_buffer(ctx, buf)
                stats.consume_s += time.monotonic() - t0
                stats.done_reqs += 1
            finally:
                req.consumer.close()
                await budget.release(cost)

        tasks = [asyncio.create_task(handle(r)) for r in ordered]
        reporter = asyncio.create_task(_report_progress(stats, rank, "read"))
        try:
            results = await asyncio.gather(*tasks, return_exceptions=True)
            errors = [r for r in results if isinstance(r, BaseException)]
            if errors:
                raise errors[0]
            for path, (total, ranges) in partial_sums.items():
                want = checksums.get(path) if checksums else None
                want_len = checksums.get(integrity.len_key(path)) if checksums else None
                if not want or not want_len:
                    continue
                ranges.sort()
                covered = 0
                for s, e in ranges:
                    if s != covered:
                        covered = -1
                        break
                    covered = e
                if covered != int(want_len):
                    continue
                got = "psum64:" + format(total, "016x")
                if got != want:
                    raise RuntimeError(
                        f"checksum mismatch for tiled read of '{path}': "
                        f"snapshot recorded {want}, read back {got} — the "
                        "file is corrupted or was modified after the "
                        "snapshot was committed"
                    )
        finally:
            reporter.cancel()
            executor.shutdown(wait=False)
            try:
                await storage.close_for_loop()
            except Exception:
                logger.exception("storage close at pipeline end failed")

    return _spawn_pipeline(main, stats, staged_event, done_event)


def sync_execute_read_reqs(
    read_reqs: List[ReadReq],
    storage: StoragePlugin,
    memory_budget_bytes: int,
    rank: int,
    checksums: Optional[dict] = None,
) -> ExecutionStats:
    pending = execute_read_reqs(
        read_reqs, storage, memory_budget_bytes, rank, checksums
    )
    pending.complete()
    import os

    if os.environ.get("TSAMD_TIMING"):
        s = pending.stats
        wall = (s.end_ts or 0) - s.begin_ts
        print(
            f"[tsamd timing] read: wall={wall:.2f}s reqs={s.total_reqs} "
            f"bytes={s.io_bytes/1e9:.2f}GB io_busy={s.io_s:.2f}s "
            f"consume_busy={s.consume_s:.2f}s"
        )
    if rank == 0 and pending.stats.io_bytes:
        logger.info(
            "Read %.1f MB in %.2fs (%.2f GB/s)",
            pending.stats.io_bytes / 1e6,
            (pending.stats.end_ts or 0) - pending.stats.begin_ts,
            pending.stats.throughput_bytes_per_sec() / 1e9,
        )
    return pending.stats


async def _report_progress(stats: ExecutionStats, rank: int, verb: str) -> None:
    if rank != 0:
        return
    interval = 10.0
    while True:
        await asyncio.sleep(interval)
        logger.info(
            "[rank %d] %s progress: %d/%d reqs, %.1f MB staged, %.1f MB io",
            rank,
            verb,
            stats.done_reqs,
            stats.total_reqs,
            stats.staged_bytes / 1e6,
            stats.io_bytes / 1e6,
        )
```

### torchsnapshot_amd/storage/fs.py

```python

from __future__ import annotations

import asyncio
import errno
import os
import shutil
import stat
from concurrent.futures import ThreadPoolExecutor
from typing import List, Optional, Set

from .. import knobs
from ..io_types import ReadIO, StoragePlugin, WriteIO

try:
    from torchsnapshot_amd import _csnap
except ImportError:
    _csnap = None


def _fsync_enabled() -> bool:
    return os.environ.get("TSAMD_FSYNC", "0") not in ("0", "", "false")


def _as_u8_mv(buf) -> memoryview:
    mv = memoryview(buf)
    if mv.format != "B":
        mv = mv.cast("B")
    return mv


REUSE_MIN_BYTES = 1 << 20


def _fsync_file_and_dir(fd: int, full: str) -> None:
    os.fsync(fd)
    dfd = os.open(os.path.dirname(full) or ".", os.O_RDONLY)
    try:
        os.fsync(dfd)
    finally:
        os.close(dfd)


def _write_file_py(
    full: str, buf, fsync: bool, chunk_bytes: int, reuse: bool
) -> bool:
    if chunk_bytes <= 0:
        raise ValueError("chunk_bytes must be positive")
    mv = _as_u8_mv(buf)
    total = len(mv)
    fd = -1
    old_size = 0
    reused = False
    if reuse and total >= REUSE_MIN_BYTES:
        try:
            fd = os.open(full, os.O_WRONLY)
        except FileNotFoundError:
            fd = -1
        if fd >= 0:
            try:
                st = os.fstat(fd)
            except BaseException:
                os.close(fd)
                raise
            if stat.S_ISREG(st.st_mode):
                old_size = st.st_size
                reused = True
            else:
                os.close(fd)
                fd = -1
    if fd < 0:
        fd = os.open(full, os.O_WRONLY | os.O_CREAT | os.O_TRUNC, 0o644)
    try:
        off = 0
        while off < total:
            n = os.pwrite(fd, mv[off : off + chunk_bytes], off)
            if n == 0:
                raise OSError(errno.EIO, os.strerror(errno.EIO), full)
            off += n
        if reused and old_size > total:
            os.ftruncate(fd, total)
        if fsync:
            _fsync_file_and_dir(fd, full)
    finally:
        os.close(fd)
    return reused


def _write_file_native(
    full: str, buf, fsync: bool, chunk_bytes: int, reuse: bool
) -> bool:
    return _csnap.file_write(
        full, buf, fsync=fsync, chunk_bytes=chunk_bytes, reuse=reuse
    )


def write_file(
    full: str, buf, fsync: bool, chunk_bytes: int, reuse: bool
) -> bool:
    if _csnap is not None:
        return _write_file_native(full, buf, fsync, chunk_bytes, reuse)
    return _write_file_py(full, buf, fsync, chunk_bytes, reuse)


class FSStoragePlugin(StoragePlugin):
    def __init__(self, root: str, storage_options: Optional[dict] = None) -> None:
        self.root = root
        opts = storage_options or {}
        nthreads = int(opts.get("io_threads", knobs.get_max_io_concurrency()))
        self._executor = ThreadPoolExecutor(
            max_workers=nthreads, thread_name_prefix="tsamd-fs"
        )
        self._created_dirs: Set[str] = set()


    def _abspath(self, path: str) -> str:
        return os.path.join(self.root, path)

    def _ensure_dir(self, dirname: str) -> None:
        if dirname in self._created_dirs:
            return
        os.makedirs(dirname, exist_ok=True)
        self._created_dirs.add(dirname)

    def _write_sync(self, path: str, buf) -> None:
        full = self._abspath(path)
        self._ensure_dir(os.path.dirname(full))
        fsync = _fsync_enabled()
        write_file(
            full,
            buf,
            fsync=fsync,
            chunk_bytes=knobs.get_storage_write_chunk_bytes(),
            reuse=knobs.is_fs_reuse_pages_enabled() and not fsync,
        )

    def _pread_segment(
        self, full: str, mv: memoryview, file_off: int
    ) -> None:
        fd = os.open(full, os.O_RDONLY)
        try:
            try:
                os.posix_fadvise(
                    fd, file_off, len(mv), os.POSIX_FADV_SEQUENTIAL
                )
                if os.environ.get("TSAMD_FS_WILLNEED", "1") not in ("0", ""):
                    os.posix_fadvise(
                        fd, file_off, len(mv), os.POSIX_FADV_WILLNEED
                    )
            except (AttributeError, OSError):
                pass
            nbytes = len(mv)
            off = 0
            while off < nbytes:
                n = os.preadv(fd, [mv[off:]], file_off + off)
                if n == 0:
                    raise EOFError(
                        f"unexpected EOF reading {full} at offset "
                        f"{file_off + off} (wanted {nbytes} from {file_off})"
                    )
                off += n
        finally:
            os.close(fd)

    def _read_sync(self, read_io: ReadIO) -> None:
        full = self._abspath(read_io.path)
        if read_io.byte_range is None:
            start, end = 0, os.path.getsize(full)
        else:
            start, end = read_io.byte_range
        nbytes = end - start
        if read_io.buf_alloc is not None:
            buf = read_io.buf_alloc(nbytes)
        else:
            buf = bytearray(nbytes)
        self._pread_segment(full, _as_u8_mv(buf), start)
        read_io.buf = buf

    @staticmethod
    def _segments(nbytes: int) -> List[tuple]:
        seg = knobs.get_fs_io_segment_bytes()
        return [(o, min(o + seg, nbytes)) for o in range(0, nbytes, seg)]


    async def write(self, write_io: WriteIO) -> None:
        loop = asyncio.get_running_loop()
        await loop.run_in_executor(
            self._executor, self._write_sync, write_io.path, write_io.buf
        )

    async def read(self, read_io: ReadIO) -> None:
        loop = asyncio.get_running_loop()
        full = self._abspath(read_io.path)
        if read_io.byte_range is None:
            start = 0
            end = await loop.run_in_executor(None, os.path.getsize, full)
        else:
            start, end = read_io.byte_range
        nbytes = end - start
        if nbytes < knobs.get_fs_parallel_io_min_bytes():
            await loop.run_in_executor(self._executor, self._read_sync, read_io)
            return
        if read_io.buf_alloc is not None:
            buf = read_io.buf_alloc(nbytes)
        else:
            buf = bytearray(nbytes)
        mv = _as_u8_mv(buf)
        await asyncio.gather(
            *(
                loop.run_in_executor(
                    self._executor,
                    self._pread_segment,
                    full,
                    mv[s:e],
                    start + s,
                )
                for s, e in self._segments(nbytes)
            )
        )
        read_io.buf = buf

    async def delete(self, path: str) -> None:
        loop = asyncio.get_running_loop()
        await loop.run_in_executor(self._executor, os.remove, self._abspath(path))

    async def delete_dir(self, path: str) -> None:
        loop = asyncio.get_running_loop()
        await loop.run_in_executor(
            self._executor, shutil.rmtree, self._abspath(path)
        )

    async def close(self) -> None:
        self._executor.shutdown(wait=False)
```

Before: 37.61 GB/s.

## Stream staged segments to file writes as D2H copies land

Splits the device pack+D2H staging into segments (64MB by default), each with its own recorded event. The filesystem writer starts pwriting each segment as soon as its event completes instead of waiting for the whole batch, so GPU-to-host copy overlaps with file IO. Segmented ops also round-robin across up to 8 D2H streams. This adds extra kernel launches, events and sleep-poll waiting in the writer, and only runs on the sync, non-checksum path.

```diff
diff --git a/torchsnapshot_amd/batcher.py b/torchsnapshot_amd/batcher.py
--- a/torchsnapshot_amd/batcher.py
+++ b/torchsnapshot_amd/batcher.py
@@ -118,17 +118,34 @@
         loop = asyncio.get_running_loop()
         device = self.tensors[0].device
         if device.type == "cuda":
-            return await loop.run_in_executor(ctx.executor, self._stage_device)
+            return await loop.run_in_executor(
+                ctx.executor, self._stage_device, ctx
+            )
         return await loop.run_in_executor(ctx.executor, self._stage_cpu)
 
-    def _stage_device(self) -> BufferType:
+    def _stage_device(self, ctx: Optional[StageContext] = None) -> BufferType:
         from . import integrity
 
         engine = get_staging_engine(self.tensors[0].device)
         ck = integrity.checksumming_enabled()
+        seg = knobs.get_stage_segment_bytes()
+        streamed = (
+            ctx is not None
+            and not ctx.is_async
+            and not self.is_async_snapshot
+            and not ck
+            and seg > 0
+            and engine.streams_writes()
+        )
         batch = engine.stage(
-            self.tensors, compute_checksums=ck, out_dtypes=self.out_dtypes
+            self.tensors,
+            compute_checksums=ck,
+            out_dtypes=self.out_dtypes,
+            segment_bytes=seg if streamed else 0,
         )
+        if streamed and batch.handle is not None:
+            self._staged_batch = batch
+            return batch.streamed_buffer()
         batch.wait()
         if ck and batch.checksums is not None:
             total = sum(batch.checksums) % (1 << 64)
diff --git a/torchsnapshot_amd/io_preparers/tensor.py b/torchsnapshot_amd/io_preparers/tensor.py
--- a/torchsnapshot_amd/io_preparers/tensor.py
+++ b/torchsnapshot_amd/io_preparers/tensor.py
@@ -6,6 +6,7 @@
 
 import torch
 
+from .. import knobs
 from ..io_types import (
     BufferConsumer,
     BufferStager,
@@ -274,10 +275,12 @@
     async def stage_buffer(self, ctx: StageContext) -> BufferType:
         loop = asyncio.get_running_loop()
         if self.tensor.device.type == "cuda":
-            return await loop.run_in_executor(ctx.executor, self._stage_device)
+            return await loop.run_in_executor(
+                ctx.executor, self._stage_device, ctx
+            )
         return await loop.run_in_executor(ctx.executor, self._stage_cpu, ctx)
 
-    def _stage_device(self) -> BufferType:
+    def _stage_device(self, ctx: Optional[StageContext] = None) -> BufferType:
         from ..ops.staging import get_staging_engine
         from ..uvm_tensor import is_uvm_tensor, uvm_to_cpu
 
@@ -300,11 +303,24 @@
 
         engine = get_staging_engine(t.device)
         ck = integrity.checksumming_enabled()
+        seg = knobs.get_stage_segment_bytes()
+        streamed = (
+            ctx is not None
+            and not ctx.is_async
+            and not self.is_async_snapshot
+            and not ck
+            and seg > 0
+            and engine.streams_writes()
+        )
         batch = engine.stage(
             [t],
             compute_checksums=ck,
             out_dtypes=None if self.save_dtype is None else [self.save_dtype],
-        )
+            segment_bytes=seg if streamed else 0,
+        )
+        if streamed and batch.handle is not None:
+            self._staged_batch = batch
+            return batch.streamed_buffer(0)
         batch.wait()
         if ck and batch.checksums is not None:
             self.precomputed_checksum = "psum64:" + format(
diff --git a/torchsnapshot_amd/io_types.py b/torchsnapshot_amd/io_types.py
--- a/torchsnapshot_amd/io_types.py
+++ b/torchsnapshot_amd/io_types.py
@@ -4,9 +4,18 @@
 import abc
 from concurrent.futures import ThreadPoolExecutor
 from dataclasses import dataclass, field
-from typing import Any, Optional, Tuple
+from typing import Any, Callable, Optional, Tuple
 
 BufferType = Any
+
+
+@dataclass
+class StreamedBuffer:
+
+    mv: memoryview
+    nbytes: int
+    handle: int
+    wait: Callable[[], None]
 
 
 @dataclass
@@ -74,6 +83,8 @@
 
 class StoragePlugin(abc.ABC):
 
+    supports_streamed_writes: bool = False
+
     @abc.abstractmethod
     async def write(self, write_io: WriteIO) -> None:
         ...
diff --git a/torchsnapshot_amd/knobs.py b/torchsnapshot_amd/knobs.py
--- a/torchsnapshot_amd/knobs.py
+++ b/torchsnapshot_amd/knobs.py
@@ -98,6 +98,10 @@
     return _env_bytes("TSAMD_SHADOW_CPU_MAX_BYTES", 1024 * _MB)
 
 
+def get_stage_segment_bytes() -> int:
+    return max(_env_bytes("TSAMD_STAGE_SEGMENT_BYTES", 64 * _MB), 0)
+
+
 def get_storage_write_chunk_bytes() -> int:
     return _env_bytes("TSAMD_FS_WRITE_CHUNK_BYTES", 256 * _MB)
 
diff --git a/torchsnapshot_amd/ops/hip/file_sink.h b/torchsnapshot_amd/ops/hip/file_sink.h
--- a/torchsnapshot_amd/ops/hip/file_sink.h
+++ b/torchsnapshot_amd/ops/hip/file_sink.h
@@ -44,14 +44,32 @@
 
 }
 
-inline SinkResult file_write(const std::string& path, const void* data,
-                             size_t nbytes, bool do_fsync, size_t chunk_bytes,
-                             bool reuse) {
+using SegWaitFn = int (*)(void* ctx, size_t k);
+
+inline SinkResult file_write_segments(const std::string& path,
+                                      const void* data, size_t nbytes,
+                                      bool do_fsync, size_t chunk_bytes,
+                                      bool reuse, const size_t* seg_end,
+                                      size_t nseg, SegWaitFn wait_fn,
+                                      void* wait_ctx) {
   SinkResult res;
   if (chunk_bytes == 0) {
     res.err = EINVAL;
     res.op = "chunk_bytes";
     return res;
+  }
+  if (nseg == 0 || wait_fn == nullptr || seg_end == nullptr) {
+    nseg = 0;
+  } else {
+    bool ok = seg_end[nseg - 1] == nbytes;
+    for (size_t k = 1; k < nseg; ++k) {
+      ok = ok && seg_end[k - 1] <= seg_end[k];
+    }
+    if (!ok) {
+      res.err = EINVAL;
+      res.op = "seg_end";
+      return res;
+    }
   }
   int fd = -1;
   off_t old_size = 0;
@@ -89,21 +107,33 @@
 
   const char* p = static_cast<const char*>(data);
   size_t off = 0;
-  while (off < nbytes) {
-    size_t want = nbytes - off < chunk_bytes ? nbytes - off : chunk_bytes;
-    ssize_t n = ::pwrite(fd, p + off, want, static_cast<off_t>(off));
-    if (n < 0) {
-      if (errno == EINTR) continue;
-      res.err = errno;
-      res.op = "pwrite";
-      break;
+  const size_t nloops = nseg == 0 ? 1 : nseg;
+  for (size_t k = 0; k < nloops && !res.err; ++k) {
+    size_t end = nbytes;
+    if (nseg != 0) {
+      if (int rc = wait_fn(wait_ctx, k)) {
+        res.err = rc;
+        res.op = "wait";
+        break;
+      }
+      end = seg_end[k];
     }
-    if (n == 0) {
-      res.err = EIO;
-      res.op = "pwrite";
-      break;
+    while (off < end) {
+      size_t want = end - off < chunk_bytes ? end - off : chunk_bytes;
+      ssize_t n = ::pwrite(fd, p + off, want, static_cast<off_t>(off));
+      if (n < 0) {
+        if (errno == EINTR) continue;
+        res.err = errno;
+        res.op = "pwrite";
+        break;
+      }
+      if (n == 0) {
+        res.err = EIO;
+        res.op = "pwrite";
+        break;
+      }
+      off += static_cast<size_t>(n);
     }
-    off += static_cast<size_t>(n);
   }
   if (!res.err && res.reused && old_size > static_cast<off_t>(nbytes)) {
     int r;
@@ -132,4 +162,11 @@
   return res;
 }
 
+inline SinkResult file_write(const std::string& path, const void* data,
+                             size_t nbytes, bool do_fsync, size_t chunk_bytes,
+                             bool reuse) {
+  return file_write_segments(path, data, nbytes, do_fsync, chunk_bytes, reuse,
+                             nullptr, 0, nullptr, nullptr);
 }
+
+}
diff --git a/torchsnapshot_amd/ops/hip/staging.hip b/torchsnapshot_amd/ops/hip/staging.hip
--- a/torchsnapshot_amd/ops/hip/staging.hip
+++ b/torchsnapshot_amd/ops/hip/staging.hip
@@ -3,6 +3,9 @@
 #include <pybind11/pybind11.h>
 #include <pybind11/stl.h>
 
+#include <time.h>
+
+#include <algorithm>
 #include <cstdint>
 #include <cstring>
 #include <mutex>
@@ -303,9 +306,10 @@
 __global__ __launch_bounds__(kBlockThreads) void pack_kernel(
     const Desc* __restrict__ descs, int n,
     const unsigned long long* __restrict__ wu_prefix,
-    unsigned long long total_wus, char* __restrict__ flat_base,
-    unsigned long long* __restrict__ hash_out) {
-  for (unsigned long long wu = blockIdx.x; wu < total_wus; wu += gridDim.x) {
+    unsigned long long wu_begin, unsigned long long wu_end,
+    char* __restrict__ flat_base, unsigned long long* __restrict__ hash_out) {
+  for (unsigned long long wu = wu_begin + blockIdx.x; wu < wu_end;
+       wu += gridDim.x) {
     int lo = 0, hi = n - 1;
     while (lo < hi) {
       int mid = (lo + hi + 1) >> 1;
@@ -347,15 +351,16 @@
 
 
 struct DeviceCtx {
-  hipStream_t d2h_stream = nullptr;
+  std::vector<hipStream_t> d2h_streams;
+  unsigned next_d2h = 0;
   hipStream_t h2d_stream = nullptr;
   hipStream_t verify_stream = nullptr;
 };
 
 struct Op {
-  hipEvent_t ev = nullptr;
+  std::vector<hipEvent_t> evs;
+  std::vector<unsigned long long> seg_end;
   int device = 0;
-  void* scratch = nullptr;
   std::vector<char> host_staging;
 };
 
@@ -370,24 +375,61 @@
   if (it == g_ctx.end()) {
     HIP_CHECK(hipSetDevice(device));
     DeviceCtx ctx;
-    HIP_CHECK(hipStreamCreateWithFlags(&ctx.d2h_stream, hipStreamNonBlocking));
+    long nstreams = 8;
+    if (const char* env = getenv("TSAMD_D2H_STREAMS")) nstreams = atol(env);
+    nstreams = std::min(std::max(nstreams, 1l), 8l);
+    ctx.d2h_streams.resize(nstreams, nullptr);
+    for (hipStream_t& st : ctx.d2h_streams) {
+      HIP_CHECK(hipStreamCreateWithFlags(&st, hipStreamNonBlocking));
+    }
     HIP_CHECK(hipStreamCreateWithFlags(&ctx.h2d_stream, hipStreamNonBlocking));
     it = g_ctx.emplace(device, ctx).first;
   }
   return it->second;
 }
 
-long long register_op(hipEvent_t ev, int device, void* scratch,
+hipStream_t pick_d2h(DeviceCtx& ctx, bool segmented) {
+  if (!segmented) return ctx.d2h_streams[0];
+  std::lock_guard<std::mutex> lk(g_mu);
+  return ctx.d2h_streams[ctx.next_d2h++ % ctx.d2h_streams.size()];
+}
+
+long long register_op(std::vector<hipEvent_t>&& evs,
+                      std::vector<unsigned long long>&& seg_end, int device,
                       std::vector<char>&& staging) {
   std::lock_guard<std::mutex> lk(g_mu);
   long long h = g_next_handle++;
   Op op;
-  op.ev = ev;
+  op.evs = std::move(evs);
+  op.seg_end = std::move(seg_end);
   op.device = device;
-  op.scratch = scratch;
   op.host_staging = std::move(staging);
   g_ops.emplace(h, std::move(op));
   return h;
+}
+
+long long register_op(hipEvent_t ev, unsigned long long total_bytes,
+                      int device, std::vector<char>&& staging) {
+  return register_op(std::vector<hipEvent_t>{ev},
+                     std::vector<unsigned long long>{total_bytes}, device,
+                     std::move(staging));
+}
+
+void record_segment_event(std::vector<hipEvent_t>& evs, hipStream_t stream) {
+  hipEvent_t ev = nullptr;
+  hipError_t e = hipEventCreateWithFlags(&ev, hipEventDisableTiming);
+  if (e == hipSuccess) {
+    e = hipEventRecord(ev, stream);
+    if (e != hipSuccess) (void)hipEventDestroy(ev);
+  }
+  if (e != hipSuccess) {
+    (void)hipStreamSynchronize(stream);
+    for (hipEvent_t x : evs) (void)hipEventDestroy(x);
+    evs.clear();
+    throw std::runtime_error(std::string("HIP error recording segment event: ") +
+                             hipGetErrorString(e));
+  }
+  evs.push_back(ev);
 }
 
 void chain_after(hipStream_t side, uintptr_t producer_stream, int device) {
@@ -408,16 +450,22 @@
 constexpr int kRowInts = 19;
 
 std::vector<Desc> parse_descs(const std::vector<unsigned long long>& flat,
-                              int n) {
+                              int n, bool* ascending = nullptr) {
   if ((int)flat.size() != n * kRowInts) {
     throw std::runtime_error("bad descriptor array length");
   }
   std::vector<Desc> descs(n);
+  unsigned long long prev_end = 0;
+  if (ascending) *ascending = true;
   for (int i = 0; i < n; ++i) {
     const unsigned long long* r = flat.data() + i * kRowInts;
     Desc& d = descs[i];
     d.tensor_base = reinterpret_cast<const char*>(r[0]);
     d.flat_off = r[1];
+    if (ascending) {
+      if (r[1] < prev_end) *ascending = false;
+      prev_end = r[1] + r[2];
+    }
     if (r[2] >= (1ull << 32)) {
       throw std::runtime_error(
           "tensor too large for pack kernel (>=4GB); chunk it upstream");
@@ -463,12 +511,15 @@
 long long launch_pack(const std::vector<unsigned long long>& flat, int n,
                       uintptr_t slab_ptr, uintptr_t pinned_ptr,
                       unsigned long long total_bytes, uintptr_t producer_stream,
-                      int device, bool gather, uintptr_t hash_out_ptr) {
+                      int device, bool gather, uintptr_t hash_out_ptr,
+                      unsigned long long segment_bytes = 0) {
   HIP_CHECK(hipSetDevice(device));
   DeviceCtx& ctx = get_ctx(device);
-  hipStream_t stream = gather ? ctx.d2h_stream : ctx.h2d_stream;
-
-  std::vector<Desc> descs = parse_descs(flat, n);
+  hipStream_t stream =
+      gather ? pick_d2h(ctx, segment_bytes > 0) : ctx.h2d_stream;
+
+  bool ascending = true;
+  std::vector<Desc> descs = parse_descs(flat, n, &ascending);
   bool any_cast = false;
   for (const Desc& d : descs) any_cast = any_cast || d.cast != kCastNone;
   if (any_cast && !gather) {
@@ -524,32 +575,73 @@
     long v = atol(env);
     if (v > 0) grid_cap = (unsigned long long)v;
   }
-  unsigned int grid = (unsigned int)std::min<unsigned long long>(
-      total_wus == 0 ? 1 : total_wus, grid_cap);
   unsigned long long* hash_out =
       reinterpret_cast<unsigned long long*>(hash_out_ptr);
-  if (any_cast && hash_out != nullptr) {
-    hipLaunchKernelGGL((pack_kernel<true, true, true>), dim3(grid),
-                       dim3(kBlockThreads), 0, stream, d_descs, n, d_prefix,
-                       total_wus, flat_base, hash_out);
-  } else if (any_cast) {
-    hipLaunchKernelGGL((pack_kernel<true, false, true>), dim3(grid),
-                       dim3(kBlockThreads), 0, stream, d_descs, n, d_prefix,
-                       total_wus, flat_base, nullptr);
-  } else if (gather && hash_out != nullptr) {
-    hipLaunchKernelGGL((pack_kernel<true, true>), dim3(grid),
-                       dim3(kBlockThreads), 0, stream, d_descs, n, d_prefix,
-                       total_wus, flat_base, hash_out);
-  } else if (gather) {
-    hipLaunchKernelGGL((pack_kernel<true, false>), dim3(grid),
-                       dim3(kBlockThreads), 0, stream, d_descs, n, d_prefix,
-                       total_wus, flat_base, nullptr);
-  } else {
-    hipLaunchKernelGGL((pack_kernel<false, false>), dim3(grid),
-                       dim3(kBlockThreads), 0, stream, d_descs, n, d_prefix,
-                       total_wus, flat_base, nullptr);
-  }
-  HIP_CHECK(hipGetLastError());
+
+  std::vector<unsigned long long> seg_wu{0};
+  std::vector<unsigned long long> seg_end;
+  if (gather && direct_mode && hash_out == nullptr && segment_bytes > 0 &&
+      ascending) {
+    unsigned long long limit = segment_bytes;
+    for (int i = 0; i < n; ++i) {
+      const unsigned long long nw = wu_prefix[i + 1] - wu_prefix[i];
+      const unsigned long long off0 = descs[i].flat_off;
+      for (;;) {
+        unsigned long long j =
+            limit > off0 ? (limit - off0 + kWorkUnitBytes - 1) / kWorkUnitBytes
+                         : 0;
+        if (j >= nw) break;
+        const unsigned long long g = wu_prefix[i] + j;
+        const unsigned long long cut_off = off0 + j * kWorkUnitBytes;
+        if (g > seg_wu.back()) {
+          seg_wu.push_back(g);
+          seg_end.push_back(cut_off);
+        }
+        limit = cut_off + segment_bytes;
+      }
+    }
+  }
+  seg_wu.push_back(total_wus);
+  seg_end.push_back(total_bytes);
+
+  std::vector<hipEvent_t> evs;
+  evs.reserve(seg_end.size());
+  for (size_t k = 0; k < seg_end.size(); ++k) {
+    const unsigned long long wu_begin = seg_wu[k];
+    const unsigned long long wu_end = seg_wu[k + 1];
+    const unsigned long long seg_wus = wu_end - wu_begin;
+    unsigned int grid = (unsigned int)std::min<unsigned long long>(
+        seg_wus == 0 ? 1 : seg_wus, grid_cap);
+    if (any_cast && hash_out != nullptr) {
+      hipLaunchKernelGGL((pack_kernel<true, true, true>), dim3(grid),
+                         dim3(kBlockThreads), 0, stream, d_descs, n, d_prefix,
+                         wu_begin, wu_end, flat_base, hash_out);
+    } else if (any_cast) {
+      hipLaunchKernelGGL((pack_kernel<true, false, true>), dim3(grid),
+                         dim3(kBlockThreads), 0, stream, d_descs, n, d_prefix,
+                         wu_begin, wu_end, flat_base, nullptr);
+    } else if (gather && hash_out != nullptr) {
+      hipLaunchKernelGGL((pack_kernel<true, true>), dim3(grid),
+                         dim3(kBlockThreads), 0, stream, d_descs, n, d_prefix,
+                         wu_begin, wu_end, flat_base, hash_out);
+    } else if (gather) {
+      hipLaunchKernelGGL((pack_kernel<true, false>), dim3(grid),
+                         dim3(kBlockThreads), 0, stream, d_descs, n, d_prefix,
+                         wu_begin, wu_end, flat_base, nullptr);
+    } else {
+      hipLaunchKernelGGL((pack_kernel<false, false>), dim3(grid),
+                         dim3(kBlockThreads), 0, stream, d_descs, n, d_prefix,
+                         wu_begin, wu_end, flat_base, nullptr);
+    }
+    hipError_t lerr = hipGetLastError();
+    if (lerr != hipSuccess) {
+      (void)hipStreamSynchronize(stream);
+      for (hipEvent_t x : evs) (void)hipEventDestroy(x);
+      throw std::runtime_error(std::string("HIP error launching pack_kernel: ") +
+                               hipGetErrorString(lerr));
+    }
+    if (k + 1 < seg_end.size()) record_segment_event(evs, stream);
+  }
 
   if (gather && slab_ptr != 0) {
     HIP_CHECK(hipMemcpyAsync(reinterpret_cast<void*>(pinned_ptr),
@@ -558,10 +650,9 @@
   }
   HIP_CHECK(hipFreeAsync(scratch, stream));
 
-  hipEvent_t ev;
-  HIP_CHECK(hipEventCreateWithFlags(&ev, hipEventDisableTiming));
-  HIP_CHECK(hipEventRecord(ev, stream));
-  return register_op(ev, device, nullptr, std::move(staging));
+  record_segment_event(evs, stream);
+  return register_op(std::move(evs), std::move(seg_end), device,
+                     std::move(staging));
 }
 
 }
@@ -569,17 +660,32 @@
 
 static long long d2h_copy(uintptr_t src, uintptr_t dst_pinned,
                           unsigned long long nbytes, uintptr_t producer_stream,
-                          int device) {
+                          int device, unsigned long long segment_bytes = 0) {
   HIP_CHECK(hipSetDevice(device));
   DeviceCtx& ctx = get_ctx(device);
-  chain_after(ctx.d2h_stream, producer_stream, device);
-  HIP_CHECK(hipMemcpyAsync(reinterpret_cast<void*>(dst_pinned),
-                           reinterpret_cast<void*>(src), nbytes,
-                           hipMemcpyDeviceToHost, ctx.d2h_stream));
-  hipEvent_t ev;
-  HIP_CHECK(hipEventCreateWithFlags(&ev, hipEventDisableTiming));
-  HIP_CHECK(hipEventRecord(ev, ctx.d2h_stream));
-  return register_op(ev, device, nullptr, {});
+  hipStream_t stream = pick_d2h(ctx, segment_bytes > 0);
+  chain_after(stream, producer_stream, device);
+  const unsigned long long step =
+      segment_bytes > 0 && segment_bytes < nbytes ? segment_bytes : nbytes;
+  std::vector<hipEvent_t> evs;
+  std::vector<unsigned long long> seg_end;
+  unsigned long long off = 0;
+  do {
+    const unsigned long long len = std::min(step, nbytes - off);
+    hipError_t e = hipMemcpyAsync(reinterpret_cast<char*>(dst_pinned) + off,
+                                  reinterpret_cast<const char*>(src) + off,
+                                  len, hipMemcpyDeviceToHost, stream);
+    if (e != hipSuccess) {
+      (void)hipStreamSynchronize(stream);
+      for (hipEvent_t x : evs) (void)hipEventDestroy(x);
+      throw std::runtime_error(std::string("HIP error at hipMemcpyAsync: ") +
+                               hipGetErrorString(e));
+    }
+    record_segment_event(evs, stream);
+    off += len;
+    seg_end.push_back(off);
+  } while (off < nbytes);
+  return register_op(std::move(evs), std::move(seg_end), device, {});
 }
 
 static long long h2d_copy(uintptr_t src_pinned, uintptr_t dst,
@@ -594,16 +700,18 @@
   hipEvent_t ev;
   HIP_CHECK(hipEventCreateWithFlags(&ev, hipEventDisableTiming));
   HIP_CHECK(hipEventRecord(ev, ctx.h2d_stream));
-  return register_op(ev, device, nullptr, {});
+  return register_op(ev, nbytes, device, {});
 }
 
 static long long pack_d2h(const std::vector<unsigned long long>& flat, int n,
                           uintptr_t slab_ptr, uintptr_t pinned_ptr,
                           unsigned long long total_bytes,
                           uintptr_t producer_stream, int device,
-                          uintptr_t hash_out_ptr = 0) {
+                          uintptr_t hash_out_ptr = 0,
+                          unsigned long long segment_bytes = 0) {
   return launch_pack(flat, n, slab_ptr, pinned_ptr, total_bytes,
-                     producer_stream, device, true, hash_out_ptr);
+                     producer_stream, device, true, hash_out_ptr,
+                     segment_bytes);
 }
 
 static long long scatter_h2d(const std::vector<unsigned long long>& flat, int n,
@@ -724,10 +832,42 @@
   return total;
 }
 
-static bool file_write(py::object path, py::object buf, bool fsync,
-                       long long chunk_bytes, bool reuse) {
+
+struct SegWaitCtx {
+  std::vector<hipEvent_t> evs;
+  hipError_t hip_err = hipSuccess;
+};
+
+static int seg_wait(void* vctx, size_t k) {
+  SegWaitCtx* c = static_cast<SegWaitCtx*>(vctx);
+  if (k >= c->evs.size()) return 0;
+  for (;;) {
+    hipError_t e = hipEventQuery(c->evs[k]);
+    if (e == hipSuccess) return 0;
+    if (e != hipErrorNotReady) {
+      c->hip_err = e;
+      return (int)e;
+    }
+    struct timespec ts = {0, 150 * 1000};
+    (void)nanosleep(&ts, nullptr);
+  }
+}
+
+static bool file_write_impl(py::object path, py::object buf, bool fsync,
+                            long long chunk_bytes, bool reuse,
+                            const long long* handle) {
   if (chunk_bytes <= 0) {
     throw py::value_error("file_write: chunk_bytes must be positive");
+  }
+  SegWaitCtx wctx;
+  std::vector<unsigned long long> op_ends;
+  if (handle != nullptr) {
+    std::lock_guard<std::mutex> lk(g_mu);
+    auto it = g_ops.find(*handle);
+    if (it != g_ops.end()) {
+      wctx.evs = it->second.evs;
+      op_ends = it->second.seg_end;
+    }
   }
   PyObject* fs_bytes = nullptr;
   if (!PyUnicode_FSConverter(path.ptr(), &fs_bytes)) {
@@ -740,19 +880,58 @@
   if (PyObject_GetBuffer(buf.ptr(), &view, PyBUF_SIMPLE) != 0) {
     throw py::error_already_set();
   }
+  std::vector<size_t> seg_end;
+  for (unsigned long long e : op_ends) {
+    seg_end.push_back((size_t)std::min<unsigned long long>(e, (size_t)view.len));
+  }
+  if (!seg_end.empty() && seg_end.back() != (size_t)view.len) {
+    PyBuffer_Release(&view);
+    throw py::value_error(
+        "file_write_op: buffer is longer than the bytes the op stages");
+  }
   tsamd::SinkResult res;
   {
     py::gil_scoped_release release;
-    res = tsamd::file_write(cpath, view.buf, (size_t)view.len, fsync,
-                            (size_t)chunk_bytes, reuse);
+    if (seg_end.empty()) {
+      res = tsamd::file_write(cpath, view.buf, (size_t)view.len, fsync,
+                              (size_t)chunk_bytes, reuse);
+    } else {
+      res = tsamd::file_write_segments(
+          cpath, view.buf, (size_t)view.len, fsync, (size_t)chunk_bytes, reuse,
+          seg_end.data(), seg_end.size(), &seg_wait, &wctx);
+    }
   }
   PyBuffer_Release(&view);
+  if (res.err && wctx.hip_err != hipSuccess) {
+    throw std::runtime_error(
+        std::string("file_write_op: HIP error while waiting for a segment: ") +
+        hipGetErrorString(wctx.hip_err));
+  }
   if (res.err) {
     errno = res.err;
     PyErr_SetFromErrnoWithFilenameObject(PyExc_OSError, path.ptr());
     throw py::error_already_set();
   }
   return res.reused;
+}
+
+static bool file_write(py::object path, py::object buf, bool fsync,
+                       long long chunk_bytes, bool reuse) {
+  return file_write_impl(path, buf, fsync, chunk_bytes, reuse, nullptr);
+}
+
+static bool file_write_op(py::object path, py::object buf, long long handle,
+                          bool fsync, long long chunk_bytes, bool reuse) {
+  return file_write_impl(path, buf, fsync, chunk_bytes, reuse, &handle);
+}
+
+static std::vector<unsigned long long> op_segment_ends(long long handle) {
+  std::lock_guard<std::mutex> lk(g_mu);
+  auto it = g_ops.find(handle);
+  if (it == g_ops.end()) {
+    throw std::runtime_error("segment_ends: unknown or already waited handle");
+  }
+  return it->second.seg_end;
 }
 
 static void op_wait(long long handle) {
@@ -762,7 +941,7 @@
     std::lock_guard<std::mutex> lk(g_mu);
     auto it = g_ops.find(handle);
     if (it == g_ops.end()) return;
-    ev = it->second.ev;
+    ev = it->second.evs.back();
     device = it->second.device;
   }
   hipError_t e;
@@ -774,7 +953,7 @@
     std::lock_guard<std::mutex> lk(g_mu);
     auto it = g_ops.find(handle);
     if (it != g_ops.end()) {
-      (void)hipEventDestroy(it->second.ev);
+      for (hipEvent_t x : it->second.evs) (void)hipEventDestroy(x);
       g_ops.erase(it);
     }
   }
@@ -788,7 +967,7 @@
   std::lock_guard<std::mutex> lk(g_mu);
   auto it = g_ops.find(handle);
   if (it == g_ops.end()) return true;
-  return hipEventQuery(it->second.ev) == hipSuccess;
+  return hipEventQuery(it->second.evs.back()) == hipSuccess;
 }
 
 static bool is_managed_ptr(uintptr_t ptr) {
@@ -840,14 +1019,19 @@
 
 PYBIND11_MODULE(_csnap, m) {
   m.doc() = "torchsnapshot_amd HIP staging engine (gfx950)";
-  m.def("d2h_copy", &d2h_copy, "async D2H copy on the side stream");
+  m.def("d2h_copy", &d2h_copy,
+        "async D2H copy on the side stream; segment_bytes > 0 splits it into "
+        "one copy and one event per segment",
+        py::arg("src"), py::arg("dst_pinned"), py::arg("nbytes"),
+        py::arg("producer_stream"), py::arg("device"),
+        py::arg("segment_bytes") = 0);
   m.def("h2d_copy", &h2d_copy, "async H2D copy on the side stream");
   m.def("pack_d2h", &pack_d2h,
         "gather-pack tensors into a slab and copy it to pinned host memory",
         py::arg("flat"), py::arg("n"), py::arg("slab_ptr"),
         py::arg("pinned_ptr"), py::arg("total_bytes"),
         py::arg("producer_stream"), py::arg("device"),
-        py::arg("hash_out_ptr") = 0);
+        py::arg("hash_out_ptr") = 0, py::arg("segment_bytes") = 0);
   m.def("scatter_h2d", &scatter_h2d,
         "copy pinned host bytes to device and scatter into strided tensors");
   m.def("psum64_host", &psum64_host,
@@ -862,6 +1046,16 @@
         "existing file of >= 1 MiB payload in place instead of truncating",
         py::arg("path"), py::arg("buf"), py::arg("fsync") = false,
         py::arg("chunk_bytes") = 256ll * 1024 * 1024, py::arg("reuse") = true);
+  m.def("file_write_op", &file_write_op,
+        "file_write of an op's pinned destination that follows the op's "
+        "segments as they land (GIL released; waiting writers sleep-poll). "
+        "The op stays registered: call wait(handle) afterwards",
+        py::arg("path"), py::arg("buf"), py::arg("handle"),
+        py::arg("fsync") = false,
+        py::arg("chunk_bytes") = 256ll * 1024 * 1024, py::arg("reuse") = true);
+  m.def("segment_ends", &op_segment_ends,
+        "flat-side end offset of each segment of an op, ascending; the last "
+        "is the op's total bytes");
   m.def("wait", &op_wait, "block until an op completes");
   m.def("query", &op_query, "poll an op");
   m.def("is_managed_ptr", &is_managed_ptr);
diff --git a/torchsnapshot_amd/ops/staging.py b/torchsnapshot_amd/ops/staging.py
--- a/torchsnapshot_amd/ops/staging.py
+++ b/torchsnapshot_amd/ops/staging.py
@@ -9,6 +9,7 @@
 import torch
 
 from .. import knobs
+from ..io_types import StreamedBuffer
 
 ALIGN = 256
 
@@ -342,6 +343,15 @@
     _sources: Optional[Sequence[torch.Tensor]] = None
     _done: bool = False
 
+    @property
+    def handle(self) -> Optional[int]:
+        return self._handle
+
+    def segment_ends(self) -> List[int]:
+        if self._handle is None:
+            return [self.total_bytes]
+        return [int(e) for e in _csnap.segment_ends(self._handle)]
+
     def wait(self) -> None:
         if self._done:
             return
@@ -367,8 +377,21 @@
         assert self._done
         return memoryview(self.pinned.tensor.numpy())[: self.total_bytes]
 
+    def streamed_buffer(self, index: Optional[int] = None) -> StreamedBuffer:
+        assert self._handle is not None, "nothing in flight to stream"
+        if index is None:
+            n = self.total_bytes
+        else:
+            assert self.offsets[index] == 0
+            n = self.nbytes_list[index]
+        mv = memoryview(self.pinned.tensor.numpy())[:n]
+        return StreamedBuffer(mv=mv, nbytes=n, handle=self._handle, wait=self.wait)
+
     def release(self) -> None:
-        get_pinned_pool().release(self.pinned)
+        try:
+            self.wait()
+        finally:
+            get_pinned_pool().release(self.pinned)
 
 
 class StagingEngine:
@@ -385,6 +408,7 @@
         tensors: Sequence[torch.Tensor],
         compute_checksums: bool = False,
         out_dtypes: Optional[Sequence[Optional[torch.dtype]]] = None,
+        segment_bytes: int = 0,
     ) -> StagedBatch:
         tensors = [
             t
@@ -416,6 +440,7 @@
                 self._stage_ext(
                     tensors, items, batch, total,
                     compute_checksums=compute_checksums,
+                    segment_bytes=segment_bytes,
                 )
             else:
                 self._stage_torch_fallback(tensors, items, batch, out_dtypes)
@@ -424,6 +449,9 @@
             raise
         return batch
 
+    def streams_writes(self) -> bool:
+        return self._use_ext
+
 
     def _stage_ext(
         self,
@@ -432,6 +460,7 @@
         batch: StagedBatch,
         total: int,
         compute_checksums: bool = False,
+        segment_bytes: int = 0,
     ) -> None:
         dev_index = self.device.index or 0
         with torch.cuda.device(dev_index):
@@ -449,6 +478,7 @@
                     items[0].nbytes,
                     cur_stream,
                     dev_index,
+                    segment_bytes,
                 )
             else:
                 mode = _pack_mode()
@@ -487,6 +517,7 @@
                     cur_stream,
                     dev_index,
                     hash_ptr,
+                    segment_bytes,
                 )
                 batch._device_slab = slab
             batch._handle = handle
diff --git a/torchsnapshot_amd/scheduler.py b/torchsnapshot_amd/scheduler.py
--- a/torchsnapshot_amd/scheduler.py
+++ b/torchsnapshot_amd/scheduler.py
@@ -13,7 +13,15 @@
 import psutil
 
 from . import knobs
-from .io_types import ReadIO, ReadReq, StageContext, StoragePlugin, WriteIO, WriteReq
+from .io_types import (
+    ReadIO,
+    ReadReq,
+    StageContext,
+    StoragePlugin,
+    StreamedBuffer,
+    WriteIO,
+    WriteReq,
+)
 from .pg_wrapper import PGWrapper
 from .roctx import roctx_range
 from . import integrity
@@ -66,6 +74,8 @@
     begin_ts: float = field(default_factory=time.monotonic)
     staged_ts: Optional[float] = None
     end_ts: Optional[float] = None
+    begin_cpu: float = field(default_factory=time.process_time)
+    end_cpu: Optional[float] = None
 
     def throughput_bytes_per_sec(self) -> float:
         end = self.end_ts or time.monotonic()
@@ -134,11 +144,16 @@
 
         if os.environ.get("TSAMD_TIMING") and self.stats.staged_bytes:
             s = self.stats
-            wall = (s.end_ts or 0) - s.begin_ts
+            end = s.end_ts or 0
+            wall = end - s.begin_ts
+            staged_ts = s.staged_ts if s.staged_ts is not None else end
+            cpu = (s.end_cpu or s.begin_cpu) - s.begin_cpu
             print(
                 f"[tsamd timing] pipeline: wall={wall:.2f}s reqs={s.total_reqs} "
                 f"staged={s.staged_bytes/1e9:.2f}GB stage_busy={s.stage_s:.2f}s "
-                f"io_busy={s.io_s:.2f}s consume_busy={s.consume_s:.2f}s"
+                f"io_busy={s.io_s:.2f}s consume_busy={s.consume_s:.2f}s "
+                f"staged_at=+{staged_ts - s.begin_ts:.3f}s "
+                f"tail={end - staged_ts:.3f}s cpu={cpu:.2f}s"
             )
 
     def done(self) -> bool:
@@ -161,6 +176,7 @@
             exc_holder.append(e)
         finally:
             stats.end_ts = time.monotonic()
+            stats.end_cpu = time.process_time()
             staged_event.set()
             done_event.set()
 
@@ -216,7 +232,15 @@
                     with roctx_range(f"tsamd:stage:{req.path}"):
                         buf = await req.stager.stage_buffer(ctx)
                     stats.stage_s += time.monotonic() - t0
-                nbytes = memoryview(buf).nbytes
+                if isinstance(buf, StreamedBuffer):
+                    nbytes = buf.nbytes
+                    if not getattr(storage, "supports_streamed_writes", False):
+                        await asyncio.get_running_loop().run_in_executor(
+                            executor, buf.wait
+                        )
+                        buf = buf.mv
+                else:
+                    nbytes = memoryview(buf).nbytes
                 if do_checksum:
                     pre = getattr(req.stager, "precomputed_checksum", None)
                     if pre is not None:
diff --git a/torchsnapshot_amd/storage/fs.py b/torchsnapshot_amd/storage/fs.py
--- a/torchsnapshot_amd/storage/fs.py
+++ b/torchsnapshot_amd/storage/fs.py
@@ -10,7 +10,7 @@
 from typing import List, Optional, Set
 
 from .. import knobs
-from ..io_types import ReadIO, StoragePlugin, WriteIO
+from ..io_types import ReadIO, StoragePlugin, StreamedBuffer, WriteIO
 
 try:
     from torchsnapshot_amd import _csnap
@@ -103,6 +103,8 @@
 
 
 class FSStoragePlugin(StoragePlugin):
+    supports_streamed_writes = True
+
     def __init__(self, root: str, storage_options: Optional[dict] = None) -> None:
         self.root = root
         opts = storage_options or {}
@@ -126,6 +128,16 @@
         full = self._abspath(path)
         self._ensure_dir(os.path.dirname(full))
         fsync = _fsync_enabled()
+        if isinstance(buf, StreamedBuffer):
+            _csnap.file_write_op(
+                full,
+                buf.mv,
+                buf.handle,
+                fsync=fsync,
+                chunk_bytes=knobs.get_storage_write_chunk_bytes(),
+                reuse=knobs.is_fs_reuse_pages_enabled() and not fsync,
+            )
+            return
         write_file(
             full,
             buf,
```

Result: faster. 41.47 GB/s (median of 3 runs) (+10.3%).
